# tchamp1912/Spittle

Measured on AMD Instinct MI355X. Metric: RTFx (audio-sec/wall-sec) Whisper-large-v3 30s chunks @1/2/4/8 MI355X, higher is better.
Workload: dtype bf16; 1 GPU; whisper-large-v3 30s chunks, batch 8/GPU, greedy en, 4-token prompt + 128 decode steps, host PCM in, text out; model=synthetic:large-v3, global_batch=8, seq_len=1500, decode_steps=128, parallelism=replicas x1 (utterance shards)

## Files before the change

include/spittle_hip.h:

```cpp
#ifndef SPITTLE_HIP_H
#define SPITTLE_HIP_H

#include <stddef.h>
#include <stdint.h>

#ifdef __cplusplus
extern "C" {
#endif

#define SPT_ABI_VERSION 14

typedef enum {
    SPT_OK = 0,
    SPT_ERR_INVALID_ARG = 1,
    SPT_ERR_LOAD = 2,
    SPT_ERR_DEVICE = 3,
    SPT_ERR_OOM = 4,
    SPT_ERR_UNSUPPORTED = 5,
    SPT_ERR_INTERNAL = 6
} spt_status;

typedef enum {
    SPT_DTYPE_F32 = 0, SPT_DTYPE_BF16 = 1,
    SPT_DTYPE_F16 = 2 ,
// ... 101 lines not shown
    int32_t decoder_passes;
    int32_t beam_steps;
    int32_t encoder_windows;
    double device_ms;
    double encoder_ms;
    double decode_ms;
    int32_t pd_passes;
    int32_t pd_fallbacks;
} spt_call_stats;

spt_status spt_get_call_stats(const spt_ctx* ctx, spt_call_stats* s);
spt_status spt_get_xq_stats(const spt_ctx* ctx, int32_t* fused_launches, int32_t* fallbacks);

spt_status spt_weights_export(spt_ctx* ctx, void* dev_dst, size_t bytes);
spt_status spt_weights_import(spt_ctx* ctx, const void* dev_src, size_t bytes);
spt_status spt_weights_arena(spt_ctx* ctx, void** dev_ptr, size_t* bytes);
spt_status spt_weights_commit(spt_ctx* ctx);

spt_status spt_ctx_create_replicas(const char* model_spec, const spt_model_params* params, const int32_t* devices,
                                   int32_t n_devices, spt_ctx** out, double* bcast_ms, char* err, size_t errlen);
spt_status spt_transcribe_batch_replicas(spt_ctx* const* ctxs, int32_t n_ctx, const float* const* pcm,
                                         const size_t* n_samples, size_t batch, const spt_infer_params* params,
                                         spt_result** out);

typedef enum {
    SPT_PROBE_DEC_CROSS_ATTN = 0,
    SPT_PROBE_DEC_SELF_ATTN = 1,
    SPT_PROBE_DEC_LOGITS = 2,
    SPT_PROBE_DEC_FC1 = 3,
    SPT_PROBE_ENC_FC1_GEMM = 4,
    SPT_PROBE_ENC_ATTN = 5
} spt_probe_kind;
spt_status spt_probe_kernel(spt_ctx* ctx, int32_t kind, int32_t iters, double* avg_us, double* work,
                            int32_t* work_is_flops);

spt_status spt_debug_mel(spt_ctx* ctx, const float* pcm16k, size_t n_samples, float* out);
spt_status spt_debug_mel_at(spt_ctx* ctx, const float* pcm16k, size_t n_samples, int32_t seek, float* out);
spt_status spt_debug_encode(spt_ctx* ctx, const float* mel, float* out);
spt_status spt_debug_weight_checksum(spt_ctx* ctx, int32_t tensor_id, double* out2);
spt_status spt_debug_ggml_tokenize(const char* model_path, const char* text, int32_t* tokens, int32_t n_max,
                                   int32_t* n_out);
spt_status spt_debug_ggml_dequant(int32_t ggml_type, const void* src, int64_t n, float* dst);
typedef struct {
    float temperature;
    int32_t suppress_blank;
    int32_t no_ts;
    int32_t max_initial;
    int32_t n_max;
    int32_t max_tokens;
    uint64_t seed;
} spt_sample_params;
spt_status spt_debug_sample_tokens(int32_t device, int32_t dtype, const float* logits, int32_t n_steps, int32_t B,
                                   int32_t n_vocab, int32_t ldl, int32_t eot, int32_t beg, int32_t blank,
                                   const uint32_t* suppress, const spt_sample_params* prm, const int32_t* seek,
                                   const int32_t* seek_end, int32_t* state, int32_t* done, const int32_t* forced,
                                   int32_t forced_len, int32_t out_cap, int32_t* dec_state, int32_t Tq, int32_t d,
                                   int32_t ctx, const float* emb, const float* pos, int32_t* out_tok, float* out_plog,
                                   float* out_tid, int32_t* next_tok, float* x, uint32_t* arrive, char* err,
                                   size_t errlen);
spt_status spt_debug_sample_beam(int32_t device, const float* logits, int32_t B, int32_t n_vocab, int32_t ldl,
                                 int32_t eot, int32_t beg, int32_t blank, const uint32_t* suppress,
                                 const spt_sample_params* prm, const int32_t* row, int32_t step, int32_t k,
                                 int32_t chunked, int32_t* cand_id, float* cand_lp, int32_t* tid, char* err,
                                 size_t errlen);
spt_status spt_debug_sample_kv_gather(int32_t device, int32_t dtype, const float* src, float* dst,
                                      const int32_t* rows, int32_t L, int32_t B, int32_t H, int32_t ctx,
                                      int32_t pos0, char* err, size_t errlen);
spt_status spt_debug_attn_enc(int32_t device, int32_t dtype, const float* qkv, int32_t B, int32_t T, int32_t H,
                              float* out, char* err, size_t errlen);
spt_status spt_debug_attn_self(int32_t device, int32_t dtype, const float* q, const float* cache, int32_t B,
                               int32_t H, int32_t ctx, int32_t Tq, int32_t pos0, float* out, char* err,
                               size_t errlen);
enum {
    SPT_ATTN_CROSS_8WAVE = 0,
    SPT_ATTN_CROSS_VW = 1,
    SPT_ATTN_CROSS_VW_PQ = 2,
    SPT_ATTN_CROSS_VW_MERGE = 3,
    SPT_ATTN_CROSS_VW_PQ_MERGE = 4
};
spt_status spt_debug_attn_cross(int32_t device, int32_t dtype, int32_t mode, const float* q, const float* k,
                                const float* v, float pad_value, int32_t B, int32_t B_layout, int32_t b0, int32_t H,
                                int32_t T_enc, int32_t Tq, int32_t splits, const int32_t* kvrow, int32_t share,
                                float* out, float* part, char* err, size_t errlen);

#define SPT_HAS_QUANT_RESIDENT 1
spt_status spt_get_weight_residency(const spt_ctx* ctx, int64_t* resident_weights, int64_t* resident_bytes,
                                    int32_t* ggml_type);
enum { SPT_GGML_Q4_1 = 3, SPT_GGML_Q5_0 = 6, SPT_GGML_Q5_1 = 7 };
enum { SPT_GV_BIAS = 0, SPT_GV_BIAS_GELU = 1, SPT_GV_PARTIAL = 2, SPT_GV_QKV_CACHE = 3, SPT_GV_LOGITS = 4,
       SPT_GV_BIAS_RESID = 5 };
enum { SPT_QGEMV_A_DIRECT = 0, SPT_QGEMV_A_LN = 1 };
spt_status spt_debug_qgemv(int32_t device, int32_t dtype, int32_t ggml_type, const void* blocks, size_t blocks_bytes,
                           int32_t N, int32_t K, const float* act, int32_t R, const float* ln_w, const float* ln_b,
                           const float* bias, const float* resid, int32_t mode, int32_t a_src, int32_t ksplit,
                           float* out_plain, float* out_packed, float* top_plain, float* top_packed, float* unpacked,
                           char* err, size_t errlen);

typedef struct spt_pk_ctx spt_pk_ctx;

typedef struct {
    int32_t dtype;
    int32_t device;
    int32_t max_batch;
    float max_seconds;
    uint64_t seed;
    uint32_t flags;
    int32_t reserved0;
} spt_pk_model_params;

#define SPT_PK_WEIGHTS_EMPTY 1u

typedef enum { SPT_PK_TS_TOKEN = 0, SPT_PK_TS_WORD = 1, SPT_PK_TS_SEGMENT = 2 } spt_pk_granularity;

typedef struct {
    int32_t max_symbols;
    int32_t timestamp_granularity;
} spt_pk_infer_params;

typedef struct {
    double start, end;
    char* text;
    int32_t i0, n_tokens;
} spt_pk_segment;

typedef struct {
    char* text;
    int32_t* tokens;
    int32_t* frames;
    float* logit;
    float* runner_up;
    int32_t n_tokens;
    int32_t n_segments;
    spt_pk_segment* segments;
    int32_t n_chunks;
    int32_t reserved0;
} spt_pk_result;

typedef struct {
    int32_t n_mels, d, n_layers, n_heads, ff, sub_ch, conv_k, pred, n_vocab, n_dur;
    int32_t dtype, max_batch, max_samples, reserved0;
    int64_t weight_bytes, workspace_bytes;
} spt_pk_model_info;

typedef struct {
    double mel_ms, encoder_ms, decode_ms, total_ms, h2d_ms;
    int32_t n_steps;
    int32_t batch;
    int32_t enc_frames;
    int32_t reserved0;
} spt_pk_timings;

void spt_parakeet_default_model_params(spt_pk_model_params* p);
void spt_parakeet_default_infer_params(spt_pk_infer_params* p);
spt_status spt_parakeet_create(const char* model_spec, const spt_pk_model_params* params, spt_pk_ctx** out,
                               char* err, size_t errlen);

typedef struct spt_pk_onnx spt_pk_onnx;
spt_status spt_parakeet_onnx_open(const char* dir, spt_pk_onnx** out, spt_pk_model_info* info, char* err, size_t errlen);
int64_t spt_parakeet_onnx_tensor(const spt_pk_onnx* h, int32_t tensor_id, const float** data);
int64_t spt_parakeet_onnx_qtensor(const spt_pk_onnx* h, int32_t tensor_id, const int16_t** q, const float** scales,
                                  const int32_t** zero_points, int32_t* n_scales);
const char* spt_parakeet_onnx_piece(const spt_pk_onnx* h, int32_t token_id);
void spt_parakeet_onnx_close(spt_pk_onnx* h);
void spt_parakeet_destroy(spt_pk_ctx* ctx);
const char* spt_parakeet_last_error(const spt_pk_ctx* ctx);
spt_status spt_parakeet_info(const spt_pk_ctx* ctx, spt_pk_model_info* info);
// ... 219 lines not shown
```

rust/spittle-hip-sys/src/lib.rs:

```rust
#![allow(non_camel_case_types)]

use std::os::raw::{c_char, c_int, c_void};

pub const SPT_ABI_VERSION: c_int = 14;
pub const SPT_PK_STAGE_COUNT: c_int = 9;

pub type spt_status = c_int;
pub const SPT_OK: spt_status = 0;
pub const SPT_ERR_INVALID_ARG: spt_status = 1;
pub const SPT_ERR_LOAD: spt_status = 2;
pub const SPT_ERR_DEVICE: spt_status = 3;
pub const SPT_ERR_OOM: spt_status = 4;
pub const SPT_ERR_UNSUPPORTED: spt_status = 5;
pub const SPT_ERR_INTERNAL: spt_status = 6;

pub type spt_dtype = c_int;
pub const SPT_DTYPE_F32: spt_dtype = 0;
pub const SPT_DTYPE_BF16: spt_dtype = 1;
pub const SPT_DTYPE_F16: spt_dtype = 2;
pub const SPT_DTYPE_I8: spt_dtype = 3;
pub const SPT_ATTN_CROSS_8WAVE: i32 = 0;
pub const SPT_ATTN_CROSS_VW: i32 = 1;
pub const SPT_ATTN_CROSS_VW_PQ: i32 = 2;
pub const SPT_ATTN_CROSS_VW_MERGE: i32 = 3;
// ... 288 lines not shown
    ) -> spt_status;
    pub fn spt_debug_sample_beam(
        device: i32,
        logits: *const f32,
        b: i32,
        n_vocab: i32,
        ldl: i32,
        eot: i32,
        beg: i32,
        blank: i32,
        suppress: *const u32,
        prm: *const spt_sample_params,
        row: *const i32,
        step: i32,
        k: i32,
        chunked: i32,
        cand_id: *mut i32,
        cand_lp: *mut f32,
        tid: *mut i32,
        err: *mut c_char,
        errlen: usize,
    ) -> spt_status;
    pub fn spt_debug_sample_kv_gather(
        device: i32,
        dtype: i32,
        src: *const f32,
        dst: *mut f32,
        rows: *const i32,
        l: i32,
        b: i32,
        h: i32,
        ctx: i32,
        pos0: i32,
        err: *mut c_char,
        errlen: usize,
    ) -> spt_status;
    pub fn spt_debug_attn_enc(
        device: i32,
        dtype: i32,
        qkv: *const f32,
        b: i32,
        t: i32,
        h: i32,
        out: *mut f32,
        err: *mut c_char,
        errlen: usize,
    ) -> spt_status;
    pub fn spt_debug_attn_self(
        device: i32,
        dtype: i32,
        q: *const f32,
        cache: *const f32,
        b: i32,
        h: i32,
        ctx: i32,
        tq: i32,
        pos0: i32,
        out: *mut f32,
        err: *mut c_char,
        errlen: usize,
    ) -> spt_status;
    pub fn spt_debug_attn_cross(
        device: i32,
        dtype: i32,
        mode: i32,
        q: *const f32,
        k: *const f32,
        v: *const f32,
        pad_value: f32,
        b: i32,
        b_layout: i32,
        b0: i32,
        h: i32,
        t_enc: i32,
        tq: i32,
        splits: i32,
        kvrow: *const i32,
        share: i32,
        out: *mut f32,
        part: *mut f32,
        err: *mut c_char,
        errlen: usize,
    ) -> spt_status;
    pub fn spt_get_weight_residency(
        ctx: *const spt_ctx,
        resident_weights: *mut i64,
        resident_bytes: *mut i64,
        ggml_type: *mut i32,
    ) -> spt_status;
    pub fn spt_debug_qgemv(
        device: i32,
        dtype: i32,
        ggml_type: i32,
        blocks: *const c_void,
        blocks_bytes: usize,
        n: i32,
        k: i32,
        act: *const f32,
        r: i32,
        ln_w: *const f32,
        ln_b: *const f32,
        bias: *const f32,
        resid: *const f32,
        mode: i32,
        a_src: i32,
        ksplit: i32,
        out_plain: *mut f32,
        out_packed: *mut f32,
        top_plain: *mut f32,
        top_packed: *mut f32,
        unpacked: *mut f32,
        err: *mut c_char,
        errlen: usize,
    ) -> spt_status;

    pub fn spt_parakeet_default_model_params(p: *mut spt_pk_model_params);
    pub fn spt_parakeet_default_infer_params(p: *mut spt_pk_infer_params);
    pub fn spt_parakeet_create(
        model_spec: *const c_char,
        params: *const spt_pk_model_params,
        out: *mut *mut spt_pk_ctx,
        err: *mut c_char,
        errlen: usize,
    ) -> spt_status;
    pub fn spt_parakeet_destroy(ctx: *mut spt_pk_ctx);
    pub fn spt_parakeet_last_error(ctx: *const spt_pk_ctx) -> *const c_char;
    pub fn spt_parakeet_info(ctx: *const spt_pk_ctx, info: *mut spt_pk_model_info) -> spt_status;
    pub fn spt_parakeet_tensor_numel(ctx: *const spt_pk_ctx, tensor_id: i32, n: *mut i64) -> spt_status;
    pub fn spt_parakeet_set_tensor(ctx: *mut spt_pk_ctx, tensor_id: i32, data: *const f32, n: i64) -> spt_status;
    pub fn spt_parakeet_set_vocab(ctx: *mut spt_pk_ctx, pieces: *const *const c_char, n: i32) -> spt_status;
    pub fn spt_parakeet_transcribe(
        ctx: *mut spt_pk_ctx,
        pcm16k: *const f32,
        n_samples: usize,
        params: *const spt_pk_infer_params,
        out: *mut *mut spt_pk_result,
    ) -> spt_status;
    pub fn spt_parakeet_transcribe_batch(
        ctx: *mut spt_pk_ctx,
        pcm: *const *const f32,
        n_samples: *const usize,
        batch: usize,
        params: *const spt_pk_infer_params,
        out: *mut *mut spt_pk_result,
    ) -> spt_status;
    pub fn spt_parakeet_transcribe_batch_device(
        ctx: *mut spt_pk_ctx,
        pcm_dev: *const f32,
        stride: usize,
        n_samples: *const usize,
        batch: usize,
        params: *const spt_pk_infer_params,
        out: *mut *mut spt_pk_result,
    ) -> spt_status;
    pub fn spt_parakeet_result_free(r: *mut spt_pk_result);
    pub fn spt_parakeet_get_timings(ctx: *const spt_pk_ctx, t: *mut spt_pk_timings) -> spt_status;
    pub fn spt_parakeet_profile_encoder(ctx: *mut spt_pk_ctx, iters: i32, ms: *mut f64, n: i32) -> spt_status;
    pub fn spt_parakeet_debug_mel(ctx: *mut spt_pk_ctx, pcm16k: *const f32, n_samples: usize, out: *mut f32) -> spt_status;
    pub fn spt_parakeet_debug_encode(ctx: *mut spt_pk_ctx, mel: *const f32, t: i32, out: *mut f32) -> spt_status;
    pub fn spt_parakeet_debug_last_encoder(ctx: *mut spt_pk_ctx, b: i32, out: *mut f32, t3: *mut i32) -> spt_status;
    pub fn spt_parakeet_debug_decode(
        ctx: *mut spt_pk_ctx,
        enc: *const f32,
        t3: i32,
        max_symbols: i32,
        out: *mut *mut spt_pk_result,
// ... 463 lines not shown
```

spittle_amd/_lib.py:

```python
from __future__ import annotations

import ctypes as C
import os

HERE = os.path.dirname(os.path.abspath(__file__))
LIB_PATH = os.path.join(HERE, "libspittle_hip.so")

SPT_OK, SPT_ERR_INVALID_ARG, SPT_ERR_LOAD, SPT_ERR_DEVICE, SPT_ERR_OOM, SPT_ERR_UNSUPPORTED, SPT_ERR_INTERNAL = range(7)
STATUS_NAMES = {0: "OK", 1: "INVALID_ARG", 2: "LOAD", 3: "DEVICE", 4: "OOM", 5: "UNSUPPORTED", 6: "INTERNAL"}
SPT_DTYPE_F32, SPT_DTYPE_BF16, SPT_DTYPE_F16, SPT_DTYPE_I8 = 0, 1, 2, 3
SPT_SUPPRESS_BLANK, SPT_NO_TIMESTAMPS, SPT_IGNORE_EOT, SPT_SUPPRESS_NST = 1, 2, 4, 8

EXPORTS = [
    "spt_version", "spt_default_model_params", "spt_default_infer_params", "spt_ctx_create",
    "spt_ctx_destroy", "spt_last_error", "spt_ctx_info", "spt_transcribe", "spt_transcribe_batch",
    "spt_transcribe_batch_device", "spt_result_free", "spt_get_timings", "spt_get_call_stats", "spt_get_xq_stats", "spt_debug_mel",
    "spt_debug_mel_at", "spt_debug_encode", "spt_debug_weight_checksum", "spt_probe_kernel", "spt_language_code",
    "spt_tokenize", "spt_token_to_str", "spt_debug_ggml_tokenize", "spt_debug_ggml_dequant",
    "spt_weights_export", "spt_weights_import", "spt_weights_arena", "spt_weights_commit",
    "spt_ctx_create_replicas", "spt_transcribe_batch_replicas",
    "spt_parakeet_default_model_params", "spt_parakeet_default_infer_params", "spt_parakeet_create",
    "spt_parakeet_destroy", "spt_parakeet_last_error", "spt_parakeet_info", "spt_parakeet_tensor_numel",
    "spt_parakeet_set_tensor", "spt_parakeet_set_vocab", "spt_parakeet_transcribe", "spt_parakeet_transcribe_batch",
    "spt_parakeet_transcribe_batch_device", "spt_parakeet_result_free", "spt_parakeet_get_timings",
    "spt_parakeet_debug_mel", "spt_parakeet_debug_encode", "spt_parakeet_debug_decode", "spt_parakeet_debug_last_encoder",
    "spt_parakeet_debug_weight_checksum", "spt_parakeet_onnx_open", "spt_parakeet_onnx_tensor",
    "spt_parakeet_onnx_piece", "spt_parakeet_onnx_close",
    "spt_resampler_create", "spt_resampler_info", "spt_resample_output_len", "spt_resample",
    "spt_resampler_last_error", "spt_resampler_destroy",
    "spt_vad_default_params", "spt_vad_create", "spt_vad_push", "spt_vad_result_free", "spt_vad_reset",
    "spt_vad_last_error", "spt_vad_destroy",
    "spt_parakeet_profile_encoder",
    "spt_parakeet_onnx_qtensor", "spt_parakeet_debug_qgemm", "spt_parakeet_debug_tap", "spt_parakeet_debug_tap_read",
    "spt_moonshine_default_model_params", "spt_moonshine_default_infer_params", "spt_moonshine_create",
    "spt_moonshine_destroy", "spt_moonshine_last_error", "spt_moonshine_info", "spt_moonshine_tensor_numel",
    "spt_moonshine_set_tensor", "spt_moonshine_missing_tensors", "spt_moonshine_set_vocab", "spt_moonshine_transcribe",
    "spt_moonshine_transcribe_batch", "spt_moonshine_result_free", "spt_moonshine_get_timings",
    "spt_moonshine_debug_stem", "spt_moonshine_debug_encode", "spt_moonshine_debug_logits",
    "spt_sensevoice_default_model_params", "spt_sensevoice_default_infer_params", "spt_sensevoice_create",
    "spt_sensevoice_destroy", "spt_sensevoice_last_error", "spt_sensevoice_info", "spt_sensevoice_tensor_numel",
    "spt_sensevoice_set_tensor", "spt_sensevoice_missing_tensors", "spt_sensevoice_set_cmvn",
    "spt_sensevoice_set_vocab", "spt_sensevoice_n_rows", "spt_sensevoice_transcribe",
    "spt_sensevoice_transcribe_batch", "spt_sensevoice_result_free", "spt_sensevoice_get_timings",
    "spt_sensevoice_debug_features", "spt_sensevoice_debug_encode", "spt_sensevoice_debug_frames",
    "spt_debug_sample_tokens", "spt_debug_sample_beam", "spt_debug_sample_kv_gather",
    "spt_debug_attn_enc", "spt_debug_attn_self", "spt_debug_attn_cross",
    "spt_debug_qgemv", "spt_get_weight_residency",
]
SPT_MODEL_QUANT_RESIDENT = 2
SPT_GGML_Q4_1, SPT_GGML_Q5_0, SPT_GGML_Q5_1 = 3, 6, 7
SPT_GV_BIAS, SPT_GV_BIAS_GELU, SPT_GV_PARTIAL, SPT_GV_QKV_CACHE, SPT_GV_LOGITS, SPT_GV_BIAS_RESID = range(6)
SPT_QGEMV_A_DIRECT, SPT_QGEMV_A_LN = 0, 1
SPT_ATTN_CROSS_8WAVE, SPT_ATTN_CROSS_VW, SPT_ATTN_CROSS_VW_PQ, SPT_ATTN_CROSS_VW_MERGE, SPT_ATTN_CROSS_VW_PQ_MERGE = range(5)
SPT_SV_LANG_AUTO, SPT_SV_LANG_ZH, SPT_SV_LANG_EN, SPT_SV_LANG_YUE, SPT_SV_LANG_JA, SPT_SV_LANG_KO = range(6)
SPT_PK_WEIGHTS_EMPTY = 1
SPT_PK_TS_TOKEN, SPT_PK_TS_WORD, SPT_PK_TS_SEGMENT = 0, 1, 2
SPT_MODEL_WEIGHTS_EXTERNAL = 1
PK_STAGES = ("subsampling", "pos", "layernorm", "ffn", "qkv_out", "attn", "conv_pw", "conv_dw", "joint_enc")
PROBES = {"dec_cross_attn": 0, "dec_self_attn": 1, "dec_logits": 2, "dec_fc1": 3, "enc_fc1_gemm": 4,
          "enc_attn": 5}


class ModelParams(C.Structure):
    _fields_ = [("dtype", C.c_int32), ("device", C.c_int32), ("max_batch", C.c_int32),
                ("flags", C.c_uint32), ("seed", C.c_uint64)]


class InferParams(C.Structure):
    _fields_ = [("language", C.c_char_p), ("translate", C.c_int32), ("initial_prompt", C.c_char_p),
                ("flags", C.c_uint32), ("max_new_tokens", C.c_int32), ("temperature", C.c_float),
                ("beam_size", C.c_int32), ("forced_tokens", C.POINTER(C.c_int32)), ("n_forced", C.c_int32),
                ("prompt_tokens", C.POINTER(C.c_int32)), ("n_prompt_tokens", C.c_int32),
                ("temperature_inc", C.c_float), ("best_of", C.c_int32), ("entropy_thold", C.c_float),
                ("logprob_thold", C.c_float), ("max_initial_ts", C.c_float), ("reserved0", C.c_int32),
                ("seed", C.c_uint64)]


class Segment(C.Structure):
    _fields_ = [("t0", C.c_int64), ("t1", C.c_int64), ("text", C.c_char_p), ("i0", C.c_int32),
                ("n_tokens", C.c_int32)]


class Result(C.Structure):
    _fields_ = [("text", C.c_char_p), ("tokens", C.POINTER(C.c_int32)), ("top1", C.POINTER(C.c_float)),
                ("top2", C.POINTER(C.c_float)), ("n_tokens", C.c_int32), ("n_windows", C.c_int32),
                ("language", C.c_int32), ("n_segments", C.c_int32), ("segments", C.POINTER(Segment)),
                ("n_fallbacks", C.c_int32), ("reserved0", C.c_int32)]


class ModelInfo(C.Structure):
    _fields_ = [(n, C.c_int32) for n in ("n_mels", "d", "n_head", "n_enc", "n_dec", "n_vocab", "n_audio_ctx",
                                          "n_text_ctx", "dtype", "max_batch")] + \
               [("weight_bytes", C.c_int64), ("workspace_bytes", C.c_int64)]


class Timings(C.Structure):
    _fields_ = [(n, C.c_double) for n in ("mel_ms", "encoder_ms", "cross_kv_ms", "decode_ms", "total_ms",
                                           "h2d_ms")] + [("n_decode_passes", C.c_int32), ("batch", C.c_int32)]


class CallStats(C.Structure):
    _fields_ = [(n, C.c_int32) for n in ("engine_calls", "decoder_passes", "beam_steps", "encoder_windows")] + \
               [(n, C.c_double) for n in ("device_ms", "encoder_ms", "decode_ms")] + \
               [(n, C.c_int32) for n in ("pd_passes", "pd_fallbacks")]


class PkModelParams(C.Structure):
    _fields_ = [("dtype", C.c_int32), ("device", C.c_int32), ("max_batch", C.c_int32), ("max_seconds", C.c_float),
                ("seed", C.c_uint64), ("flags", C.c_uint32), ("reserved0", C.c_int32)]


class PkInferParams(C.Structure):
    _fields_ = [("max_symbols", C.c_int32), ("timestamp_granularity", C.c_int32)]


class PkSegment(C.Structure):
    _fields_ = [("start", C.c_double), ("end", C.c_double), ("text", C.c_char_p), ("i0", C.c_int32),
                ("n_tokens", C.c_int32)]


class PkResult(C.Structure):
    _fields_ = [("text", C.c_char_p), ("tokens", C.POINTER(C.c_int32)), ("frames", C.POINTER(C.c_int32)),
                ("logit", C.POINTER(C.c_float)), ("runner_up", C.POINTER(C.c_float)), ("n_tokens", C.c_int32),
                ("n_segments", C.c_int32), ("segments", C.POINTER(PkSegment)), ("n_chunks", C.c_int32),
                ("reserved0", C.c_int32)]


class PkModelInfo(C.Structure):
    _fields_ = [(n, C.c_int32) for n in ("n_mels", "d", "n_layers", "n_heads", "ff", "sub_ch", "conv_k", "pred",
# ... 193 lines not shown
    L.spt_vad_result_free.restype = None
    L.spt_vad_reset.argtypes = [vp, C.c_int32]
    L.spt_vad_reset.restype = C.c_int
    L.spt_vad_last_error.argtypes = [vp]
    L.spt_vad_last_error.restype = C.c_char_p
    L.spt_vad_destroy.argtypes = [vp]
    L.spt_vad_destroy.restype = None
    MR = C.POINTER(C.POINTER(MsResult))
    L.spt_moonshine_default_model_params.argtypes = [C.POINTER(MsModelParams)]
    L.spt_moonshine_default_model_params.restype = None
    L.spt_moonshine_default_infer_params.argtypes = [C.POINTER(MsInferParams)]
    L.spt_moonshine_default_infer_params.restype = None
    L.spt_moonshine_create.argtypes = [C.c_char_p, C.POINTER(MsModelParams), C.POINTER(vp), C.c_char_p, C.c_size_t]
    L.spt_moonshine_destroy.argtypes = [vp]
    L.spt_moonshine_destroy.restype = None
    L.spt_moonshine_last_error.argtypes = [vp]
    L.spt_moonshine_last_error.restype = C.c_char_p
    L.spt_moonshine_info.argtypes = [vp, C.POINTER(MsModelInfo)]
    L.spt_moonshine_tensor_numel.argtypes = [vp, C.c_char_p, C.POINTER(C.c_int64)]
    L.spt_moonshine_set_tensor.argtypes = [vp, C.c_char_p, fp, C.c_int64]
    L.spt_moonshine_missing_tensors.argtypes = [vp]
    L.spt_moonshine_missing_tensors.restype = C.c_int32
    L.spt_moonshine_set_vocab.argtypes = [vp, C.POINTER(C.c_char_p), C.c_int32]
    L.spt_moonshine_transcribe.argtypes = [vp, fp, C.c_size_t, C.POINTER(MsInferParams), MR]
    L.spt_moonshine_transcribe_batch.argtypes = [vp, C.POINTER(fp), C.POINTER(C.c_size_t), C.c_size_t,
                                                 C.POINTER(MsInferParams), MR]
    L.spt_moonshine_result_free.argtypes = [C.POINTER(MsResult)]
    L.spt_moonshine_result_free.restype = None
    L.spt_moonshine_get_timings.argtypes = [vp, C.POINTER(MsTimings)]
    L.spt_moonshine_debug_stem.argtypes = [vp, fp, C.c_size_t, fp]
    L.spt_moonshine_debug_encode.argtypes = [vp, fp, C.c_size_t, fp]
    L.spt_moonshine_debug_logits.argtypes = [vp, fp, C.c_size_t, i32p, C.c_int32, fp]
    for fn in ("spt_moonshine_create", "spt_moonshine_info", "spt_moonshine_tensor_numel", "spt_moonshine_set_tensor",
               "spt_moonshine_set_vocab", "spt_moonshine_transcribe", "spt_moonshine_transcribe_batch",
               "spt_moonshine_get_timings", "spt_moonshine_debug_stem", "spt_moonshine_debug_encode",
               "spt_moonshine_debug_logits"):
        getattr(L, fn).restype = C.c_int
    SR = C.POINTER(C.POINTER(SvResult))
    svip = C.POINTER(SvInferParams)
    L.spt_sensevoice_default_model_params.argtypes = [C.POINTER(SvModelParams)]
    L.spt_sensevoice_default_model_params.restype = None
    L.spt_sensevoice_default_infer_params.argtypes = [svip]
    L.spt_sensevoice_default_infer_params.restype = None
    L.spt_sensevoice_create.argtypes = [C.c_char_p, C.POINTER(SvModelParams), C.POINTER(vp), C.c_char_p, C.c_size_t]
    L.spt_sensevoice_destroy.argtypes = [vp]
    L.spt_sensevoice_destroy.restype = None
    L.spt_sensevoice_last_error.argtypes = [vp]
    L.spt_sensevoice_last_error.restype = C.c_char_p
    L.spt_sensevoice_info.argtypes = [vp, C.POINTER(SvModelInfo)]
    L.spt_sensevoice_tensor_numel.argtypes = [vp, C.c_char_p, C.POINTER(C.c_int64)]
    L.spt_sensevoice_set_tensor.argtypes = [vp, C.c_char_p, fp, C.c_int64]
    L.spt_sensevoice_missing_tensors.argtypes = [vp]
    L.spt_sensevoice_missing_tensors.restype = C.c_int32
    L.spt_sensevoice_set_cmvn.argtypes = [vp, fp, fp, C.c_int32]
    L.spt_sensevoice_set_vocab.argtypes = [vp, C.POINTER(C.c_char_p), C.c_int32]
    L.spt_sensevoice_n_rows.argtypes = [vp, C.c_size_t]
    L.spt_sensevoice_n_rows.restype = C.c_int32
    L.spt_sensevoice_transcribe.argtypes = [vp, fp, C.c_size_t, svip, SR]
    L.spt_sensevoice_transcribe_batch.argtypes = [vp, C.POINTER(fp), C.POINTER(C.c_size_t), C.c_size_t, svip, SR]
    L.spt_sensevoice_result_free.argtypes = [C.POINTER(SvResult)]
    L.spt_sensevoice_result_free.restype = None
    L.spt_sensevoice_get_timings.argtypes = [vp, C.POINTER(SvTimings)]
    L.spt_sensevoice_debug_features.argtypes = [vp, fp, C.c_size_t, fp]
    L.spt_sensevoice_debug_encode.argtypes = [vp, fp, C.c_size_t, svip, fp]
    L.spt_sensevoice_debug_frames.argtypes = [vp, fp, C.c_size_t, svip, i32p, fp, fp]
    for fn in ("spt_sensevoice_create", "spt_sensevoice_info", "spt_sensevoice_tensor_numel", "spt_sensevoice_set_tensor",
               "spt_sensevoice_set_cmvn", "spt_sensevoice_set_vocab", "spt_sensevoice_transcribe",
               "spt_sensevoice_transcribe_batch", "spt_sensevoice_get_timings", "spt_sensevoice_debug_features",
               "spt_sensevoice_debug_encode", "spt_sensevoice_debug_frames"):
        getattr(L, fn).restype = C.c_int
    u32p, spp, i32 = C.POINTER(C.c_uint32), C.POINTER(SampleParams), C.c_int32
    L.spt_debug_sample_tokens.argtypes = [i32, i32, fp, i32, i32, i32, i32, i32, i32, i32, u32p, spp, i32p, i32p, i32p,
                                          i32p, i32p, i32, i32, i32p, i32, i32, i32, fp, fp, i32p, fp, fp, i32p, fp,
                                          u32p, C.c_char_p, C.c_size_t]
    L.spt_debug_sample_beam.argtypes = [i32, fp, i32, i32, i32, i32, i32, i32, u32p, spp, i32p, i32, i32, i32, i32p, fp,
                                        i32p, C.c_char_p, C.c_size_t]
    L.spt_debug_sample_kv_gather.argtypes = [i32, i32, fp, fp, i32p, i32, i32, i32, i32, i32, C.c_char_p, C.c_size_t]
    for fn in ("spt_debug_sample_tokens", "spt_debug_sample_beam", "spt_debug_sample_kv_gather"):
        getattr(L, fn).restype = C.c_int
    L.spt_debug_attn_enc.argtypes = [i32, i32, fp, i32, i32, i32, fp, C.c_char_p, C.c_size_t]
    L.spt_debug_attn_self.argtypes = [i32, i32, fp, fp, i32, i32, i32, i32, i32, fp, C.c_char_p, C.c_size_t]
    L.spt_debug_attn_cross.argtypes = [i32, i32, i32, fp, fp, fp, C.c_float, i32, i32, i32, i32, i32, i32, i32, i32p,
                                       i32, fp, fp, C.c_char_p, C.c_size_t]
    for fn in ("spt_debug_attn_enc", "spt_debug_attn_self", "spt_debug_attn_cross"):
        getattr(L, fn).restype = C.c_int
    L.spt_debug_qgemv.argtypes = [i32, i32, i32, C.c_void_p, C.c_size_t, i32, i32, fp, i32, fp, fp, fp, fp, i32, i32,
                                  i32, fp, fp, fp, fp, fp, C.c_char_p, C.c_size_t]
    L.spt_debug_qgemv.restype = C.c_int
    L.spt_get_weight_residency.argtypes = [vp, C.POINTER(C.c_int64), C.POINTER(C.c_int64), C.POINTER(C.c_int32)]
    L.spt_get_weight_residency.restype = C.c_int
    for fn in EXPORTS:
        if fn.startswith("spt_parakeet_") and fn not in ("spt_parakeet_default_model_params",
                                                          "spt_parakeet_default_infer_params", "spt_parakeet_destroy",
                                                          "spt_parakeet_last_error", "spt_parakeet_result_free",
                                                          "spt_parakeet_onnx_tensor", "spt_parakeet_onnx_piece",
                                                          "spt_parakeet_onnx_close", "spt_parakeet_onnx_qtensor"):
            getattr(L, fn).restype = C.c_int
    for fn in ("spt_weights_arena", "spt_weights_commit", "spt_ctx_create_replicas", "spt_transcribe_batch_replicas",
               "spt_weights_export", "spt_weights_import", "spt_ctx_info", "spt_transcribe", "spt_transcribe_batch", "spt_transcribe_batch_device",
               "spt_get_timings", "spt_get_call_stats", "spt_get_xq_stats", "spt_debug_mel", "spt_debug_mel_at", "spt_debug_encode", "spt_debug_weight_checksum",
               "spt_probe_kernel", "spt_tokenize", "spt_debug_ggml_tokenize", "spt_debug_ggml_dequant"):
        getattr(L, fn).restype = C.c_int
    _lib = L
    return L
```

spittle_amd/attn_debug.py:

```python
from __future__ import annotations

import ctypes as C

import numpy as np

from . import _lib as L
from .engine import TranscriptionError

DTYPES = {"f32": L.SPT_DTYPE_F32, "bf16": L.SPT_DTYPE_BF16, "f16": L.SPT_DTYPE_F16}
MODES = {"8wave": L.SPT_ATTN_CROSS_8WAVE, "vw": L.SPT_ATTN_CROSS_VW, "vw_pq": L.SPT_ATTN_CROSS_VW_PQ,
         "vw_merge": L.SPT_ATTN_CROSS_VW_MERGE, "vw_pq_merge": L.SPT_ATTN_CROSS_VW_PQ_MERGE}


def _ptr(x, t=C.c_float):
    return None if x is None else x.ctypes.data_as(C.POINTER(t))


def _check(st, err):
    if st != L.SPT_OK:
        raise TranscriptionError(st, err.value.decode())


def enc(qkv, B, T, H, dtype="f32", device: int = 0) -> np.ndarray:
    lib = L.load()
    x = None if qkv is None else np.ascontiguousarray(qkv, np.float32)
    if x is not None and x.size != B * T * 3 * H * 64:
        raise ValueError("enc: qkv is [B*T][3*H*64]")
    out = np.zeros((max(B * T, 1), max(H, 1) * 64), np.float32)
    err = C.create_string_buffer(512)
    _check(lib.spt_debug_attn_enc(device, DTYPES[dtype], _ptr(x), B, T, H, _ptr(out), err, 512), err)
    return out


def self_attn(q, cache, pos0, Tq, dtype="f32", device: int = 0) -> np.ndarray:
    lib = L.load()
    c = np.ascontiguousarray(cache, np.float32)
    two, B, H, ctx, hd = c.shape
    if two != 2 or hd != 64:
        raise ValueError("self_attn: cache is [2][B][H][ctx][64]")
    x = np.ascontiguousarray(q, np.float32)
    if x.size != B * max(Tq, 0) * H * 64 and 1 <= Tq <= 4:
        raise ValueError("self_attn: q is [B*Tq][H*64]")
    out = np.zeros((B * max(Tq, 1), H * 64), np.float32)
    err = C.create_string_buffer(512)
    _check(lib.spt_debug_attn_self(device, DTYPES[dtype], _ptr(x), _ptr(c), B, H, ctx, Tq, pos0, _ptr(out), err, 512),
           err)
    return out


def cross(q, k, v, *, Tq=1, mode="8wave", splits=1, b0=0, B=None, kvrow=None, share=1, pad_value=0.0, dtype="f32",
          device: int = 0) -> np.ndarray:
    lib = L.load()
    kk = np.ascontiguousarray(k, np.float32)
    vv = np.ascontiguousarray(v, np.float32)
    B_layout, H, T_enc, hd = kk.shape
    if hd != 64 or vv.shape != kk.shape:
        raise ValueError("cross: k and v are [B_layout][H][T_enc][64]")
    x = np.ascontiguousarray(q, np.float32)
    if B is None:
        B = x.size // (max(Tq, 1) * H * 64)
    if 1 <= Tq <= 4 and x.size != B * Tq * H * 64:
        raise ValueError("cross: q is [B*Tq][H*64]")
    km = None if kvrow is None else np.ascontiguousarray(kvrow, np.int32)
    if km is not None and km.shape != (B,):
        raise ValueError("cross: one window per row")
    m = MODES[mode] if isinstance(mode, str) else int(mode)
    R = max(B * max(Tq, 1), 1)
    vw = m >= L.SPT_ATTN_CROSS_VW
    want_part = (vw and m not in (L.SPT_ATTN_CROSS_VW_MERGE, L.SPT_ATTN_CROSS_VW_PQ_MERGE)) or (not vw and splits > 1)
    out = np.zeros((R, H * 64), np.float32)
    part = np.zeros((R, H, 8 if vw else max(min(splits, 4), 1), 66), np.float32)
    err = C.create_string_buffer(512)
    st = lib.spt_debug_attn_cross(device, DTYPES[dtype], m, _ptr(x), _ptr(kk), _ptr(vv), float(pad_value), B, B_layout,
                                  b0, H, T_enc, Tq, splits, _ptr(km, C.c_int32), share, _ptr(out), _ptr(part), err, 512)
    _check(st, err)
    return part if want_part else out
```

spittle_amd/csrc/capi_attn.cpp:

```cpp
#include <hip/hip_runtime.h>
#include <string.h>

#include <stdexcept>
#include <string>
#include <vector>

#include "../../include/spittle_hip.h"
#include "capi_debug.h"
#include "capi_internal.h"
#include "common.h"
#include "kernels.h"

namespace {

using namespace spt::dbg;

const void* up_as(Scope& sc, int dtype, const float* v, size_t n, std::vector<uint16_t>& h16) {
    if (dtype == spt::DT_F32) return sc.up(v, n);
    h16 = to_half_storage(dtype, v, n);
    return sc.up(h16.data(), n);
}

void down_f32(Scope& sc, int dtype, const void* dev, float* h, size_t n) {
    if (dtype == spt::DT_F32) {
// ... 89 lines not shown
    }
}

spt_status spt_debug_attn_cross(int32_t device, int32_t dtype, int32_t mode, const float* q, const float* k,
                                const float* v, float pad_value, int32_t B, int32_t B_layout, int32_t b0, int32_t H,
                                int32_t T_enc, int32_t Tq, int32_t splits, const int32_t* kvrow, int32_t share,
                                float* out, float* part, char* err, size_t errlen) {
    if (!q || !k || !v) {
        set_err(err, errlen, "null argument");
        return SPT_ERR_INVALID_ARG;
    }
    const bool vw = mode >= SPT_ATTN_CROSS_VW;
    const bool per_query = mode == SPT_ATTN_CROSS_VW_PQ || mode == SPT_ATTN_CROSS_VW_PQ_MERGE;
    const bool merge = mode == SPT_ATTN_CROSS_VW_MERGE || mode == SPT_ATTN_CROSS_VW_PQ_MERGE;
    try {
        check_dtype(dtype);
        if (mode < SPT_ATTN_CROSS_8WAVE || mode > SPT_ATTN_CROSS_VW_PQ_MERGE) throw std::runtime_error("debug_attn_cross: mode 0..4");
        if (B < 1 || B > 1024 || H < 1 || B_layout < 1) throw std::runtime_error("debug_attn_cross: need 1..1024 rows, H, B_layout >= 1");
        if (T_enc < 1) throw std::runtime_error("debug_attn_cross: T_enc below 1");
        if (Tq < 1 || Tq > 4) throw std::runtime_error("dec_cross_attn: 1..4 queries per sequence");
        if (splits < 1 || splits > 4) throw std::runtime_error("dec_cross_attn: 1..4 key chunks");
        if (splits > 1 && vw) throw std::runtime_error("debug_attn_cross: key chunks are the 8-wave kernel's");
        if (share < 1 || share > 8 || B % share) throw std::runtime_error("dec_cross_attn: rows per window 1..8, dividing B");
        if (share > 1 && !kvrow) throw std::runtime_error("dec_cross_attn: shared windows need the window map");
        if (per_query && Tq != 1) throw std::runtime_error("debug_attn_cross: per_query is the one-token step's");
        const int nq = share * Tq;
        const int NQ = nq == 1 ? 1 : Tq > 1 ? 4 : (spt::dtype_size(dtype) == 2 ? 5 : 4);
        if (splits > 1 && nq > NQ) throw std::runtime_error("dec_cross_attn: key chunks need one query chunk per window");
        if ((int64_t)((T_enc + 31) / 32) * B_layout * H * 4096 >= (int64_t)INT32_MAX)
            throw std::runtime_error("dec_cross_attn: a layer's cross K/V exceeds 2^31 elements");
        if (spt::kv_layer_elems(B_layout, H, T_enc) > kMaxElems || (int64_t)B * Tq * H * 66 * 8 > kMaxElems)
            throw std::runtime_error("debug_attn_cross: buffers above 2^26 elements");
        if (b0 < 0 || (int64_t)b0 + B / share > B_layout) throw std::runtime_error("debug_attn_cross: b0 + B / share beyond B_layout");
        if (kvrow)
            for (int i = 0; i < B; ++i)
                if (kvrow[i] < 0 || (int64_t)b0 + kvrow[i] >= B_layout)
                    throw std::runtime_error("debug_attn_cross: window map entry outside the layout");
        const bool wants_part = (vw && !merge) || (!vw && splits > 1);
        if (wants_part ? !part : !out) throw std::runtime_error("debug_attn_cross: null output for this mode");
    } catch (const std::exception& e) {
        set_err(err, errlen, e.what());
        return SPT_ERR_INVALID_ARG;
    }
    if (spt_status s = device_ok(device, err, errlen)) return s;
    try {
        const size_t n_kv = (size_t)spt::kv_layer_elems(B_layout, H, T_enc);
        std::vector<float> lay(n_kv, pad_value);
        const int T32 = (T_enc + 31) / 32 * 32;
        for (int kvi = 0; kvi < 2; ++kvi) {
            const float* src = kvi ? v : k;
            for (int b = 0; b < B_layout; ++b)
                for (int h = 0; h < H; ++h)
                    for (int t = 0; t < T32; ++t) {
                        float* dst = lay.data() + spt::kv_offset(0, kvi, b, h, t, 0, B_layout, H, T_enc);
                        if (t < T_enc) memcpy(dst, src + (((size_t)b * H + h) * T_enc + t) * 64, 64 * sizeof(float));
                    }
        }
        const size_t R = (size_t)B * Tq, nq_el = R * H * 64, esz = (size_t)spt::dtype_size(dtype);
        const int S = vw ? 8 : splits;
        const size_t n_part = R * H * S * 66;
        std::vector<uint16_t> q16, kv16;
        Scope sc(device);
        const void* d_q = up_as(sc, dtype, q, nq_el, q16);
        const char* d_kv = (const char*)up_as(sc, dtype, lay.data(), n_kv, kv16) + (size_t)b0 * H * 4096 * esz;
        const int* d_map = kvrow ? sc.up(kvrow, (size_t)B) : nullptr;
        float* d_part = (vw || splits > 1) ? sc.out<float>(n_part) : nullptr;
        void* d_out = (!vw && splits == 1) || merge ? sc.out<char>(nq_el * esz) : nullptr;
        if (vw) {
            spt::dec_cross_attn_vw(dtype, d_q, d_kv, B, B_layout, H, T_enc, Tq, d_part, sc.st, d_map, share, per_query);
            if (merge) spt::dec_attn_part_merge(dtype, d_part, (int)R, H, d_out, sc.st);
        } else {
            spt::dec_cross_attn(dtype, d_q, d_kv, B, B_layout, H, T_enc, Tq, d_out, sc.st, splits, d_part, d_map, share);
        }
        if (d_out) down_f32(sc, dtype, d_out, out, nq_el);
        else sc.down(part, (const float*)d_part, n_part);
        sc.sync();
        return SPT_OK;
    } catch (const std::exception& e) {
        set_err(err, errlen, e.what());
        return spt_classify(e);
    }
}

}
```

spittle_amd/csrc/dec_attn.h:

```cpp
#pragma once
#include "common.h"

namespace spt {
namespace {

constexpr int AW = 8;
constexpr float kLog2Scale = 0.125f * 1.4426950408889634f;

template <typename T> struct KVChunk;
template <> struct KVChunk<bf16> {
    bf16x8 v;
    __device__ __forceinline__ void load(const bf16* p) { v = *(const bf16x8*)p; }
    __device__ __forceinline__ float at(int e) const { return bf2f((bf16)v[e]); }
};
template <> struct KVChunk<f16> {
    f16x8 v;
    __device__ __forceinline__ void load(const f16* p) { v = *(const f16x8*)p; }
    __device__ __forceinline__ float at(int e) const { return (float)v[e]; }
};
template <> struct KVChunk<float> {
    f32x4 a, b;
    __device__ __forceinline__ void load(const float* p) { a = *(const f32x4*)p; b = *(const f32x4*)(p + 4); }
    __device__ __forceinline__ float at(int e) const { return e < 4 ? a[e] : b[e - 4]; }
};
// ... 68 lines not shown
#pragma unroll
                for (int e = 0; e < 8; ++e) o[t][e] = __builtin_fmaf(p, vc[i].at(e), o[t][e]);
            }
            l[t] = __builtin_fmaf(l[t], alpha, ls);
            m[t] = mn;
        }
    }
    template <int MAXB>
    __device__ __forceinline__ void run(int blk, int nblk, const float (&qv)[NQ][8], const int (&lim)[NQ], int Tq) {
        if (blk >= nblk) return;
        const int cnt = (nblk - 1 - blk) / NW + 1;
        const int mine = blk + (cnt - 1) * NW;
        if (MAXB <= 8 && cnt <= MAXB) {
#pragma unroll
            for (int d = 0; d < PF - 1 && d < MAXB; ++d) load_blk(kc_[d], vc_[d], min(blk + d * NW, mine));
#pragma unroll
            for (int i = 0; i < (MAXB <= 8 ? MAXB : 1); ++i) {
                if (i >= cnt) break;
                if (i + PF - 1 < (MAXB <= 8 ? MAXB : 1))
                    load_blk(kc_[(i + PF - 1) % PF], vc_[(i + PF - 1) % PF], min(blk + (i + PF - 1) * NW, mine));
                process(kc_[i % PF], vc_[i % PF], (blk + i * NW) * KB, qv, lim, Tq);
            }
            return;
        }
        load_blk(kc_[0], vc_[0], blk);
        while (blk < nblk) {
            load_blk(kc_[1], vc_[1], min(blk + NW, mine));
            process(kc_[0], vc_[0], blk * KB, qv, lim, Tq);
            blk += NW;
            if (blk >= nblk) break;
            load_blk(kc_[0], vc_[0], min(blk + NW, mine));
            process(kc_[1], vc_[1], blk * KB, qv, lim, Tq);
            blk += NW;
        }
    }
    template <int MAXB>
    __device__ __forceinline__ void run_pre(int blk, int nblk, const float (&qv)[NQ][8], const int (&lim)[NQ], int Tq) {
        if (blk >= nblk) return;
        const int cnt = (nblk - 1 - blk) / NW + 1;
        const int mine = blk + (cnt - 1) * NW;
        if (MAXB <= 8 && cnt <= MAXB) {
#pragma unroll
            for (int d = 1; d < PF - 1 && d < MAXB; ++d) load_blk(kc_[d], vc_[d], min(blk + d * NW, mine));
#pragma unroll
            for (int i = 0; i < (MAXB <= 8 ? MAXB : 1); ++i) {
                if (i >= cnt) break;
                if (i + PF - 1 < (MAXB <= 8 ? MAXB : 1))
                    load_blk(kc_[(i + PF - 1) % PF], vc_[(i + PF - 1) % PF], min(blk + (i + PF - 1) * NW, mine));
                process(kc_[i % PF], vc_[i % PF], (blk + i * NW) * KB, qv, lim, Tq);
            }
            return;
        }
        while (blk < nblk) {
            load_blk(kc_[1], vc_[1], min(blk + NW, mine));
            process(kc_[0], vc_[0], blk * KB, qv, lim, Tq);
            blk += NW;
            if (blk >= nblk) break;
            load_blk(kc_[0], vc_[0], min(blk + NW, mine));
            process(kc_[1], vc_[1], blk * KB, qv, lim, Tq);
            blk += NW;
        }
    }
    template <int MAXB>
    __device__ __forceinline__ void ring_fill(int blk, int nblk) {
        static_assert(MAXB <= 8, "AttnWave: ring_fill / ring_run are the unrolled schedule");
        const int cnt = blk < nblk ? (nblk - 1 - blk) / NW + 1 : 1;
        const int mine = blk + (cnt - 1) * NW;
#pragma unroll
        for (int d = 0; d < PF - 1 && d < MAXB; ++d) load_blk(kc_[d], vc_[d], min(blk + d * NW, mine));
    }
    template <int MAXB>
    __device__ __forceinline__ void ring_run(int blk, int nblk, const float (&qv)[NQ][8], const int (&lim)[NQ], int Tq) {
        if (blk >= nblk) return;
        const int cnt = (nblk - 1 - blk) / NW + 1;
        const int mine = blk + (cnt - 1) * NW;
#pragma unroll
        for (int i = 0; i < MAXB; ++i) {
            if (i >= cnt) break;
            if (i + PF - 1 < MAXB)
                load_blk(kc_[(i + PF - 1) % PF], vc_[(i + PF - 1) % PF], min(blk + (i + PF - 1) * NW, mine));
            process(kc_[i % PF], vc_[i % PF], (blk + i * NW) * KB, qv, lim, Tq);
        }
    }
    __device__ __forceinline__ void to_lds(float (*s_m)[NQ], float (*s_l)[NQ], float (*s_o)[NQ][64], int wid,
                                           int lane) {
        const int g = lane & 7;
#pragma unroll
        for (int t = 0; t < NQ; ++t) {
            float lt = l[t];
            lt += __shfl_xor(lt, 8, 64);
            lt += __shfl_xor(lt, 16, 64);
            lt += __shfl_xor(lt, 32, 64);
#pragma unroll
            for (int e = 0; e < 8; ++e) {
                float v = o[t][e];
                v += __shfl_xor(v, 8, 64);
                v += __shfl_xor(v, 16, 64);
                v += __shfl_xor(v, 32, 64);
                o[t][e] = v;
            }
            if (lane < 8) {
#pragma unroll
                for (int e = 0; e < 8; ++e) s_o[wid][t][8 * g + e] = o[t][e];
            }
            if (lane == 0) {
                s_m[wid][t] = m[t];
                s_l[wid][t] = lt;
            }
        }
    }
};

template <int NQ, int NW = AW>
__device__ __forceinline__ void attn_merge(const float (*s_m)[NQ], const float (*s_l)[NQ], const float (*s_o)[NQ][64],
                                           int t, int e, float& M, float& L, float& O) {
#pragma clang fp contract(off)
    M = -INFINITY;
#pragma unroll
    for (int w = 0; w < NW; ++w) M = fmaxf(M, s_m[w][t]);
    L = 0.f;
    O = 0.f;
#pragma unroll
    for (int w = 0; w < NW; ++w) {
        if (s_m[w][t] == -INFINITY) continue;
        const float f = exp2f(s_m[w][t] - M);
        L = __builtin_fmaf(s_l[w][t], f, L);
        O = __builtin_fmaf(s_o[w][t][e], f, O);
    }
}

}
}
```

spittle_amd/csrc/engine.cpp:

```cpp
#include "engine.h"
#include "ggml_file.h"
#include "ggml_qpack.h"

#include <cstdio>

#include <math.h>
#include <string.h>

#include <algorithm>
#include <functional>
#include <cstdlib>
#include <sstream>
#include <stdexcept>

#include "common.h"

namespace spt {

bool parse_synthetic_spec(const std::string& spec, ModelDims* dm, uint64_t* seed, std::string* err) {
    const std::string pfx = "synthetic:";
    if (spec.compare(0, pfx.size(), pfx) != 0) return false;
    std::vector<std::string> parts;
    std::stringstream ss(spec.substr(pfx.size()));
    std::string tok;
// ... 874 lines not shown
}

void Engine::run_cross_kv(int B) {
    const int d = dm_.d, T = dm_.n_audio_ctx;
    GemmArgs g{};
    g.A = enc_out_; g.lda = d; g.W = ckv_w_; g.ldw = d; g.M = B * T; g.N = dm_.n_dec * 2 * d; g.K = d;
    g.bias = ckv_b_; g.C = ckv_; g.kv_B = B; g.kv_T = T; g.kv_H = dm_.n_head;
    gemm_nt(dt_, EPI_KVSPLIT, g, 1, st_);
}

void Engine::enqueue_decoder_pass(DecGroup& g, int E, int Tq, const DecodeRequest& rq, int out_cap) {
    float* x = enqueue_layers(g, E, Tq);
    enqueue_head(g, Tq, rq, out_cap, x, suppress_, (rq.flags & 1u) != 0);
}

float* Engine::enqueue_layers(DecGroup& g, int E, int Tq) {
    const int d = dm_.d, H = dm_.n_head, ctx = dm_.n_text_ctx, T = dm_.n_audio_ctx, B = g.B, R = B * Tq;
    const int64_t self_layer = (int64_t)2 * B * H * ctx * 64, cross_layer = kv_layer_elems(E, H, T);
    const bool mapped = g.share > 0;
    const int runs = B / std::max(1, g.share);
    const int vw_env = getenv("SPT_XATTN_VW") ? atoi(getenv("SPT_XATTN_VW")) : 1;
    const bool vw = vw_env == 2 || (vw_env != 0 && runs * H < 96);
    const bool per_query = vw && Tq == 1 && vw_env != 3;
    const bool vw_merge = vw && R > 1;
    const int xs = vw ? (vw_merge ? 1 : 8) : mapped ? 1 : xsplit_;
    const int ks = esz_ == 2 ? 128 : 64;
    hipStream_t st = g.st;
    const bool fuse = xq_on_ && probe_kind_ < 0 && Tq == 1 && !vw && !mapped && xs == 1 && dm_.n_dec <= 64 &&
                      dec_xq_fused_ok(dt_, B, d, H, T, n_cu_);
    xq_enq_ = fuse ? dm_.n_dec : 0;
    if (fuse) {
        hipStreamCaptureStatus cap = hipStreamCaptureStatusNone;
        HIP_CHECK(hipStreamIsCapturing(st, &cap));
        if (cap == hipStreamCaptureStatusNone) cs_.xq_fused += xq_enq_;
    }
    float* xc = g.dx;
    float* xo = g.dx2;
    int np = 0;
    pend_fold_ = !getenv("SPT_DEC_XFOLD") || atoi(getenv("SPT_DEC_XFOLD")) != 0;
    auto ln_input = [&](GemvArgs& a) {
        ln_source(a, xc, g.pend, np, (int64_t)R * d);
        a.x_out = np > 0 ? xo : nullptr;
    };
    auto consumed = [&] {
        if (np > 0) std::swap(xc, xo);
        np = 0;
    };
    auto pmark = [&](int kind, int l, int which) {
        if (probe_kind_ == kind) HIP_CHECK(hipEventRecord(probe_ev_[2 * l + which], st));
    };
    auto partial = [&](GemvArgs& a, int split) {
        a.C = g.pend; a.ldc = d; a.c_split = (int64_t)R * d;
        a.ksplit = split;
        a.p_resid = pend_fold_ ? xc : nullptr;
        if (a.K / ks < split) throw std::runtime_error("decoder projection too narrow for its K split");
        np = split;
    };
    for (int l = 0; l < dm_.n_dec; ++l) {
        const DecL& e = dec_[l];
        void* skv_l = (char*)g.skv + self_layer * l * esz_;
        const void* ckv_l = (const char*)ckv_ + (cross_layer * l + (mapped ? 0 : (int64_t)g.b0 * H * 4096)) * esz_;
        {
            GemvArgs a{};
            ln_input(a); a.lda = d; a.ln_w = e.ln1_w; a.ln_b = e.ln1_b; a.R = R;
            a.W = e.qkv_w; a.wq = e.qkv_q; a.N = 3 * d; a.K = d; a.bias = e.qkv_b; a.C = g.dq; a.ldc = d;
            a.cache = skv_l; a.cache_B = B; a.cache_H = H; a.cache_ctx = ctx; a.Tq = Tq; a.st = g.ds;
            gemv(dt_, GV_QKV_CACHE, A_LN, a, st);
            consumed();
            pmark(1, l, 0);
            dec_self_attn(dt_, g.dq, skv_l, B, H, ctx, Tq, g.ds, g.dao, st);
            pmark(1, l, 1);
        }
        GemvArgs a{};
        a.A = g.dao; a.lda = d; a.R = R; a.W = e.so_w; a.wq = e.so_q; a.N = d; a.K = d; a.bias = e.so_b;
        a.C = xc; a.ldc = d;
        gemv(dt_, GV_BIAS_RESID, A_DIRECT, a, st);
        a = GemvArgs{};
        ln_input(a); a.lda = d; a.ln_w = e.ln2_w; a.ln_b = e.ln2_b; a.R = R;
        a.W = e.cq_w; a.wq = e.cq_q; a.N = d; a.K = d; a.bias = e.cq_b; a.C = g.dq; a.ldc = d;
        if (fuse) {
            if (np != 0) throw std::runtime_error("fused cross-Q launch: pending slabs before LN2");
            XqFuseArgs x{};
            x.kv = ckv_l; x.B_layout = E; x.H = H; x.T_enc = T; x.out = g.dao; x.gran = g.xq_gran; x.ds = g.ds;
            x.err = xq_err_; x.layer = l;
            dec_xq_fused(dt_, a, x, B, st);
        } else {
            gemv(dt_, GV_BIAS, A_LN, a, st);
        }
        consumed();
        pmark(0, l, 0);
        if (fuse) {
        } else if (vw) {
            dec_cross_attn_vw(dt_, g.dq, ckv_l, B, E, H, T, Tq, g.xpart, st, mapped ? g.kvrow : nullptr,
                              mapped ? g.share : 1, per_query);
            if (vw_merge) dec_attn_part_merge(dt_, g.xpart, R, H, g.dao, st);
        }
        else
            dec_cross_attn(dt_, g.dq, ckv_l, B, E, H, T, Tq, g.dao, st, xs, g.xpart, mapped ? g.kvrow : nullptr,
                           mapped ? g.share : 1);
        pmark(0, l, 1);
        a = GemvArgs{};
        a.A = g.dao; a.lda = d; a.R = R; a.W = e.co_w; a.wq = e.co_q; a.N = d; a.K = d; a.bias = e.co_b; a.C = xc; a.ldc = d;
        if (xs > 1) { a.apart = g.xpart; a.a_splits = xs; a.a_heads = H; }
        gemv(dt_, GV_BIAS_RESID, xs > 1 ? A_ATTN : A_DIRECT, a, st);
        a = GemvArgs{};
        ln_input(a); a.lda = d; a.ln_w = e.ln3_w; a.ln_b = e.ln3_b; a.R = R;
        a.W = e.fc1_w; a.wq = e.fc1_q; a.N = 4 * d; a.K = d; a.bias = e.fc1_b; a.C = g.dff; a.ldc = 4 * d;
        pmark(3, l, 0);
        gemv(dt_, GV_BIAS_GELU, A_LN, a, st);
        pmark(3, l, 1);
        consumed();
        a = GemvArgs{};
        a.A = g.dff; a.lda = 4 * d; a.R = R; a.W = e.fc2_w; a.wq = e.fc2_q; a.N = d; a.K = 4 * d; a.bias = e.fc2_b;
        partial(a, fc2_split_);
        gemv(dt_, GV_PARTIAL, A_DIRECT, a, st);
    }
    return xc;
}

void Engine::ln_source(GemvArgs& a, float* xc, float* pend, int np, int64_t slab) const {
    const int f = np > 0 && pend_fold_ ? 1 : 0;
    a.A = f ? pend : xc;
    for (int p = 0; p < kMaxPend; ++p) a.pend[p] = p < np - f ? pend + (int64_t)(p + f) * slab : zero_;
    a.n_pend = np - f;
}

void Engine::enqueue_head(DecGroup& g, int Tq, const DecodeRequest& rq, int out_cap, float* xc,
                          const uint32_t* sup, bool blank) {
    const int d = dm_.d, ctx = dm_.n_text_ctx, B = g.B, R = B * Tq;
    hipStream_t st = g.st;
    const Specials sp = specials_for(dm_.n_vocab);
    const int n_tiles = (dm_.n_vocab + 15) / 16;
    GemvArgs a{};
    ln_source(a, xc, g.pend, fc2_split_, (int64_t)R * d);
    a.lda = Tq * d; a.a_row0 = (Tq - 1) * d; a.ln_w = lnf_w_; a.ln_b = lnf_b_; a.R = B;
    a.W = tok_emb_; a.wq = tok_q_; a.N = dm_.n_vocab; a.K = d; a.C = g.logits; a.ldc = dm_.n_vocab; a.st = g.ds;
    a.suppress = sup;
    a.blank0 = blank ? sp.eot : -1;
    a.blank1 = blank ? 220 : -1;
    a.part = g.part; a.n_tiles = n_tiles;
    gemv(dt_, GV_LOGITS, A_LN, a, st);
    if (rq.beam_k > 0) {
        BeamArgs bm{};
        bm.logits = g.logits; bm.ldl = dm_.n_vocab;
        bm.n_vocab = dm_.n_vocab; bm.eot = sp.eot; bm.beg = sp.beg; bm.blank = rq.blank_tok;
        bm.suppress = sup; bm.prm = g.prm; bm.row = g.beam_row; bm.step = g.beam_step; bm.k = rq.beam_k;
        bm.cand_id = g.cand_id; bm.cand_lp = g.cand_lp; bm.tid = g.beam_tid;
        static const bool one_wg = getenv("SPT_BEAM_ONE_WG") != nullptr;
        bm.stat = one_wg ? nullptr : g.beam_stat;
        dec_beam_topk(bm, B, st);
        dec_advance(g.ds, Tq, st);
        return;
    }
    if (rq.full) {
        TsArgs t{};
        t.logits = g.logits; t.ldl = dm_.n_vocab;
        t.n_vocab = dm_.n_vocab; t.eot = sp.eot; t.beg = sp.beg; t.blank = rq.blank_tok;
        t.suppress = sup; t.prm = g.prm; t.seek = g.seek; t.seek_end = g.seek_end; t.state = g.ts_state;
        t.forced = rq.n_forced > 0 ? g.forced : nullptr; t.forced_len = rq.n_forced;
        t.next_tok = g.tok_in; t.out_tok = g.out_tok; t.out_plog = g.out_t1; t.out_tid = g.out_t2; t.out_cap = out_cap;
        t.done = g.done;
        t.emb = tok_emb_; t.emb_q = tok_q_; t.pos = dec_pos_; t.d = d; t.ctx = ctx; t.Tq = Tq; t.x = g.dx;
        t.ds = g.ds; t.arrive = g.arrive; t.stat = g.ts_stat;
        dec_ts_stats(t, B, st);
        dec_finalize_ts(dt_, t, B, st);
        return;
    }
// ... 148 lines not shown
            ~XqRestore() { on = v; }
        } xq_restore{xq_on_, xq_on};
        for (DecGroup* g : act) {
            reset_outputs(*g);
            upload_tokens(*g, [&](int, int) { return sp.sot; }, 1);
            dec_embed(dt_, g->tok_in, g->B, 1, dm_.d, tok_emb_, tok_q_, dec_pos_, g->ds, g->dx, g->st);
            float* x = enqueue_layers(*g, E, 1);
            enqueue_head(*g, 1, dq, out_cap, x, suppress_lang_, false);
        }
        std::vector<int> first((size_t)B * out_cap);
        for (DecGroup* g : act) {
            HIP_CHECK(hipMemcpyAsync(first.data() + (size_t)g->b0 * out_cap, g->out_tok, (size_t)g->B * out_cap * 4,
                                     hipMemcpyDeviceToHost, g->st));
            HIP_CHECK(hipStreamSynchronize(g->st));
        }
        for (int b = 0; b < B; ++b) {
            const int v = rq.lang_tok[b];
            lang[b] = v >= 0 ? v : first[(size_t)(-v - 1) * out_cap];
            if (lang[b] <= sp.sot || lang[b] > sp.sot + sp.n_langs) throw std::runtime_error("language detection failed");
        }
    } else if (!rq.lang_tok.empty()) {
        for (int b = 0; b < B; ++b) lang[b] = rq.lang_tok[b];
    }
    if (lang_out)
        for (int b = 0; b < B; ++b) lang_out[b] = lang[b] >= 0 ? lang[b] : (Tq >= 3 ? rq.prompt[1] : -1);
    for (DecGroup* gp : act) {
        DecGroup& g = *gp;
        reset_outputs(g);
        const bool rows = !rq.row_prefix.empty();
        const int P = rows ? (int)rq.row_prefix[0].size() : (int)rq.prefix.size();
        for (int c0 = 0; c0 < P; c0 += cmax) {
            const int n = std::min(cmax, P - c0);
            upload_tokens(g, [&](int b, int t) { return rows ? rq.row_prefix[b][c0 + t] : rq.prefix[c0 + t]; }, n);
            dec_embed(dt_, g.tok_in, g.B * n, n, dm_.d, tok_emb_, tok_q_, dec_pos_, g.ds, g.dx, g.st);
            enqueue_layers(g, E, n);
            dec_advance(g.ds, n, g.st);
        }
        auto prompt_tok = [&](int b, int t) { return (t == 1 && lang[b] >= 0) ? lang[b] : rq.prompt[t]; };
        for (int c0 = 0; c0 < Tq - Tq_head; c0 += cmax) {
            const int n = std::min(cmax, Tq - Tq_head - c0);
            upload_tokens(g, [&](int b, int t) { return prompt_tok(b, c0 + t); }, n);
            dec_embed(dt_, g.tok_in, g.B * n, n, dm_.d, tok_emb_, tok_q_, dec_pos_, g.ds, g.dx, g.st);
            enqueue_layers(g, E, n);
            dec_advance(g.ds, n, g.st);
        }
        upload_tokens(g, [&](int b, int t) { return prompt_tok(b, Tq - Tq_head + t); }, Tq_head);
        dec_embed(dt_, g.tok_in, g.B * Tq_head, Tq_head, dm_.d, tok_emb_, tok_q_, dec_pos_, g.ds, g.dx, g.st);
        if (rq.beam_k > 0) {
            beam_host_.assign((size_t)g.B * 4 + 1, 0);
            for (int b = 0; b < g.B; ++b) beam_host_[b * 4 + 3] = 3000;
            HIP_CHECK(hipMemcpyAsync(g.beam_row, beam_host_.data(), (size_t)g.B * 16, hipMemcpyHostToDevice, g.st));
            HIP_CHECK(hipMemcpyAsync(g.beam_step, beam_host_.data() + (size_t)g.B * 4, 4, hipMemcpyHostToDevice, g.st));
        }
        enqueue_decoder_pass(g, E, Tq_head, rq, out_cap);
    }
    if (rq.beam_k > 0) {
        tm_.n_decode_passes = 1;
        for (DecGroup* g : act) {
            HIP_CHECK(hipEventRecord(g->ev, g->st));
            HIP_CHECK(hipStreamWaitEvent(st_, g->ev, 0));
        }
        return;
    }
    int passes = 1;
    static const bool no_graph = getenv("SPT_NO_GRAPH") != nullptr;
    static const bool sync_debug = getenv("SPT_DEBUG_SYNC") != nullptr;
    if (rq.n_steps > 1 && no_graph) {
        for (int s = 1; s < rq.n_steps; ++s, ++passes)
            for (DecGroup* g : act) {
                enqueue_decoder_pass(*g, E, 1, rq, out_cap);
                if (!sync_debug) continue;
                const hipError_t e = hipStreamSynchronize(g->st);
                DecState h{};
                if (e == hipSuccess) HIP_CHECK(hipMemcpy(&h, g->ds, sizeof(h), hipMemcpyDeviceToHost));
                if (e != hipSuccess || h.step != s + 1 || (s % 16) == 0)
                    fprintf(stderr, "[spt] pass %d: %s step=%d pos0=%d\n", s, hipGetErrorString(e), h.step, h.pos0);
                if (e != hipSuccess) throw HipError(std::string("pass failed: ") + hipGetErrorString(e));
            }
    } else if (rq.n_steps > 1) {
        std::vector<PassGraph> ex;
        for (DecGroup* g : act) {
            GraphKey key{g->B, E, g->b0, out_cap, rq.n_forced, rq.flags, rq.full};
            key.share = S;
            key.fuse = xq_on_;
            auto it = g->graphs.find(key);
            if (it == g->graphs.end()) {
                hipGraph_t graph;
                HIP_CHECK(hipStreamBeginCapture(g->st, hipStreamCaptureModeThreadLocal));
                enqueue_decoder_pass(*g, E, 1, rq, out_cap);
                HIP_CHECK(hipStreamEndCapture(g->st, &graph));
                hipGraphExec_t exec;
                HIP_CHECK(hipGraphInstantiate(&exec, graph, nullptr, nullptr, 0));
                HIP_CHECK(hipGraphDestroy(graph));
                it = g->graphs.emplace(key, PassGraph{exec, xq_enq_}).first;
            }
            ex.push_back(it->second);
        }
        const bool early_exit = !(rq.flags & 4u);
        std::vector<int> hdone(B);
        for (int s = 1; s < rq.n_steps; ++s) {
            for (size_t i = 0; i < act.size(); ++i) {
                HIP_CHECK(hipGraphLaunch(ex[i].exec, act[i]->st));
                cs_.xq_fused += ex[i].fused;
            }
            ++passes;
            if (early_exit && (s % 16) == 0) {
                bool all = true;
                for (DecGroup* g : act) {
                    HIP_CHECK(hipMemcpyAsync(hdone.data(), g->done, g->B * 4, hipMemcpyDeviceToHost, g->st));
                    HIP_CHECK(hipStreamSynchronize(g->st));
                    all = all && std::all_of(hdone.begin(), hdone.begin() + g->B, [](int v) { return v != 0; });
                }
                if (all) break;
            }
        }
    }
    tm_.n_decode_passes = passes;
    for (DecGroup* g : act) {
        const size_t off = (size_t)g->b0 * out_cap, n = (size_t)g->B * out_cap * 4;
        HIP_CHECK(hipMemcpyAsync(tokens + off, g->out_tok, n, hipMemcpyDeviceToHost, g->st));
        if (top1) HIP_CHECK(hipMemcpyAsync(top1 + off, g->out_t1, n, hipMemcpyDeviceToHost, g->st));
        if (top2) HIP_CHECK(hipMemcpyAsync(top2 + off, g->out_t2, n, hipMemcpyDeviceToHost, g->st));
        if (ts_state_out && rq.full)
            HIP_CHECK(hipMemcpyAsync(ts_state_out + (size_t)g->b0 * 4, g->ts_state, (size_t)g->B * 16,
                                     hipMemcpyDeviceToHost, g->st));
        HIP_CHECK(hipEventRecord(g->ev, g->st));
        HIP_CHECK(hipStreamWaitEvent(st_, g->ev, 0));
    }
}

void Engine::decode(int B, const DecodeRequest& rq, int* tokens, float* top1, float* top2, int* lang_out,
                    int* ts_state_out) {
    select();
    require_weights();
    const char* xq_env = getenv("SPT_XQ_FUSE");
    xq_on_ = rq.beam_k == 0 && !(xq_env && atoi(xq_env) == 0);
    struct XqOff {
        bool& on;
        ~XqOff() { on = false; }
    } xq_off{xq_on_};
    const int fused0 = cs_.xq_fused;
    HIP_CHECK(hipEventRecord(ev_[6], st_));
    run_decode(B, rq, tokens, top1, top2, lang_out, ts_state_out);
    HIP_CHECK(hipEventRecord(ev_[7], st_));
    HIP_CHECK(hipStreamSynchronize(st_));
    HIP_CHECK(hipGetLastError());
    if (cs_.xq_fused > fused0) {
        unsigned err = 0;
        HIP_CHECK(hipMemcpy(&err, xq_err_, 4, hipMemcpyDeviceToHost));
        const char* force = getenv("SPT_XQ_FUSE_FORCE_FALLBACK");
        if (err || (force && atoi(force) != 0)) {
            HIP_CHECK(hipMemset(xq_err_, 0, 4));
            xq_on_ = false;
            cs_.xq_fallbacks++;
            HIP_CHECK(hipEventRecord(ev_[6], st_));
            run_decode(B, rq, tokens, top1, top2, lang_out, ts_state_out);
            HIP_CHECK(hipEventRecord(ev_[7], st_));
            HIP_CHECK(hipStreamSynchronize(st_));
            HIP_CHECK(hipGetLastError());
        }
    }
    tm_.batch = B;
    cs_.engine_calls++;
    cs_.decoder_passes += tm_.n_decode_passes;
    finish_call_timing();
}

void Engine::finish_call_timing() {
    float ms;
    HIP_CHECK(hipEventElapsedTime(&ms, ev_[6], ev_[7]));
    tm_.decode_ms = ms;
    double total = ms;
    if (enc_pending_) {
        float m_norm, m_enc, m_kv;
        HIP_CHECK(hipEventElapsedTime(&m_norm, ev_[2], ev_[3]));
        HIP_CHECK(hipEventElapsedTime(&m_enc, ev_[3], ev_[4]));
        HIP_CHECK(hipEventElapsedTime(&m_kv, ev_[4], ev_[5]));
        tm_.encoder_ms = m_enc;
        tm_.cross_kv_ms = m_kv;
        tm_.mel_ms = m_norm;
        cs_.encoder_ms += m_enc;
        total += m_norm + m_enc + m_kv;
    } else {
        tm_.encoder_ms = tm_.cross_kv_ms = tm_.mel_ms = 0.0;
    }
    if (mel_pending_) {
        HIP_CHECK(hipEventElapsedTime(&ms, ev_[0], ev_[1]));
        tm_.mel_ms += ms;
        total += ms;
    }
    tm_.total_ms = total;
    cs_.device_ms += total;
    cs_.decode_ms += tm_.decode_ms;
    mel_pending_ = enc_pending_ = false;
}

void Engine::transcribe_device(const float* pcm_dev, int64_t stride, const int* n_samples, int B,
                               const DecodeRequest& rq, int* tokens, float* top1, float* top2, int* lang_out,
                               int* ts_state_out) {
    if (B < 1 || B > max_batch_) throw std::runtime_error("batch exceeds the context's max_batch");
    for (int b = 0; b < B; ++b)
        if (n_samples[b] < 0 || n_samples[b] > 480000 || (int64_t)n_samples[b] > stride)
            throw std::runtime_error("each window must hold 0..480000 samples within its stride");
    load_utterances_device(pcm_dev, stride, n_samples, B);
    std::vector<int> utt(B), seek(B, 0);
    for (int b = 0; b < B; ++b) utt[b] = b;
    encode_windows(utt.data(), seek.data(), B);
    decode(B, rq, tokens, top1, top2, lang_out, ts_state_out);
}

void Engine::transcribe_host(const float* const* pcm, const int* n_samples, int B, const DecodeRequest& rq,
                             int* tokens, float* top1, float* top2, int* lang_out, int* ts_state_out) {
    if (B < 1 || B > max_batch_) throw std::runtime_error("batch exceeds the context's max_batch");
    for (int b = 0; b < B; ++b)
        if (n_samples[b] < 0 || n_samples[b] > 480000) throw std::runtime_error("window longer than 30 s");
    load_utterances(pcm, n_samples, B);
    std::vector<int> utt(B), seek(B, 0);
    for (int b = 0; b < B; ++b) utt[b] = b;
    encode_windows(utt.data(), seek.data(), B);
// ... 329 lines not shown
```

spittle_amd/csrc/engine.h:

```cpp
#pragma once
#include <hip/hip_runtime.h>
#include <stdint.h>

#include <map>
#include <set>
#include <string>
#include <vector>

#include "kernels.h"
#include "vocab.h"

namespace spt {

class GgmlFile;

struct ModelDims {
    std::string name;
    int n_mels = 80, d = 384, n_head = 6, n_enc = 4, n_dec = 4, n_vocab = 51864;
    int n_audio_ctx = 1500, n_text_ctx = 448;
};


struct DecodeRequest {
    std::vector<int> prompt;
// ... 6 lines not shown
    bool full = false;
    TsParams ts{};
    std::vector<int> seek, seek_end;
    std::vector<std::vector<int>> row_prefix;
    std::vector<int> extra_suppress;
    int blank_tok = 220;
    int beam_k = 0;
    std::vector<int> kv_row;
};

struct BeamCands {
    std::vector<int> id;
    std::vector<float> lp;
    std::vector<int> tid;
};

struct Timings {
    double mel_ms = 0, encoder_ms = 0, cross_kv_ms = 0, decode_ms = 0, total_ms = 0, h2d_ms = 0;
    int n_decode_passes = 0, batch = 0;
};

struct CallStats {
    int engine_calls = 0, decoder_passes = 0, beam_steps = 0, encoder_windows = 0;
    int pd_passes = 0;
    int pd_fallbacks = 0;
    int xq_fused = 0;
    int xq_fallbacks = 0;
    double device_ms = 0, encoder_ms = 0, decode_ms = 0;
};

class Engine {
public:
    Engine(const ModelDims& dm, int dtype, int device, int max_batch, uint64_t seed, const GgmlFile* src = nullptr,
           bool external_weights = false, bool quant_resident = false);
    ~Engine();
    Engine(const Engine&) = delete;
    Engine& operator=(const Engine&) = delete;

    const ModelDims& dims() const { return dm_; }
    int dtype() const { return dt_; }
    int max_batch() const { return max_batch_; }
    int max_rows() const { return max_rows_; }
    int64_t weight_bytes() const { return wbytes_; }
    void weight_residency(int64_t* weights, int64_t* bytes, int* type) const {
        *weights = res_weights_; *bytes = res_bytes_; *type = res_type_;
    }
    bool weights_ready() const { return weights_ready_; }
    void export_weights(void* dev_dst, int64_t bytes);
    void import_weights(const void* dev_src, int64_t bytes);
    void* weight_arena() const { return warena_; }
    int device() const { return dev_; }
    void commit_weights();
    int64_t workspace_bytes() const { return abytes_; }
    const Timings& timings() const { return tm_; }
    const CallStats& call_stats() const { return cs_; }
    void reset_call_stats() { cs_ = CallStats(); }

    void load_utterances(const float* const* pcm_host, const int* n, int U);
    void load_utterances_device(const float* pcm_dev, int64_t stride, const int* n, int U);
    void encode_windows(const int* utt, const int* seek, int E);
    int encoded_windows() const { return enc_E_; }
    void decode(int B, const DecodeRequest& rq, int* tokens, float* top1, float* top2, int* lang_out = nullptr,
                int* ts_state_out = nullptr);

    void transcribe_device(const float* pcm_dev, int64_t stride, const int* n_samples, int B, const DecodeRequest& rq,
                           int* tokens, float* top1, float* top2, int* lang_out = nullptr, int* ts_state_out = nullptr);
    void transcribe_host(const float* const* pcm, const int* n_samples, int B, const DecodeRequest& rq, int* tokens,
                         float* top1, float* top2, int* lang_out = nullptr, int* ts_state_out = nullptr);

    void beam_begin(int B, const DecodeRequest& rq, BeamCands* out, int* lang_out);
    void beam_next(const int* src, const int* tokens, const int* rowstate, int step, BeamCands* out);

    void debug_mel(const float* pcm_host, int n, int seek, float* out_host);
    void debug_encode(const float* mel_host, float* out_host);
    bool debug_weight_checksum(int tid, double* out2);
    double probe(int kind, int iters, double* work, int* is_flops);

private:
    struct GraphKey {
        int B, B_total, b0, out_cap, n_forced;
        uint32_t flags;
        bool full;
        int share = 0;
        bool fuse = false;
        bool operator<(const GraphKey& o) const {
            if (full != o.full) return full < o.full;
            if (fuse != o.fuse) return fuse < o.fuse;
            if (B != o.B) return B < o.B;
            if (share != o.share) return share < o.share;
            if (B_total != o.B_total) return B_total < o.B_total;
            if (b0 != o.b0) return b0 < o.b0;
            if (out_cap != o.out_cap) return out_cap < o.out_cap;
            if (n_forced != o.n_forced) return n_forced < o.n_forced;
            return flags < o.flags;
        }
    };
    struct PassGraph {
        hipGraphExec_t exec;
        int fused;
    };
    struct DecGroup {
        hipStream_t st = nullptr;
        hipEvent_t ev = nullptr;
        int b0 = 0, B = 0;
        float* dx = nullptr;
        void *dq = nullptr, *dao = nullptr, *dff = nullptr;
        void* skv = nullptr;
        float* logits = nullptr;
        void* part = nullptr;
        unsigned* arrive = nullptr;
        int *tok_in = nullptr, *out_tok = nullptr, *done = nullptr, *forced = nullptr;
        float *out_t1 = nullptr, *out_t2 = nullptr;
        DecState* ds = nullptr;
        float* dx2 = nullptr;
        float* pend = nullptr;
        float* xpart = nullptr;
        int *seek = nullptr, *seek_end = nullptr, *ts_state = nullptr;
        float* ts_stat = nullptr;
        float* beam_stat = nullptr;
        TsParams* prm = nullptr;
        int *beam_row = nullptr, *beam_step = nullptr, *beam_src = nullptr;
        int *cand_id = nullptr, *beam_tid = nullptr;
        float* cand_lp = nullptr;
        int* kvrow = nullptr;
        int share = 0;
        unsigned long long* xq_gran = nullptr;
        std::map<GraphKey, PassGraph> graphs;
        std::vector<int> host_tok;
        size_t host_used = 0;
    };

    void select() const;
    void release();
    void alloc_weights();
    void generate_weights();
    void load_ggml(const GgmlFile& f);
    void alloc_workspace();
    void upload_tables(const std::vector<float>* filters);
    void run_mel_utts(const float* pcm, const std::vector<int64_t>& pcm_off, const int* n, int U);
    void upload_windows(const int* utt, const int* seek, int E);
    void finish_call_timing();
    void run_encoder(int B);
    void enc_layer(int l, int Bg, int64_t r0, hipStream_t s, int probe = 0, hipEvent_t e0 = nullptr,
                   hipEvent_t e1 = nullptr);
    int enc_groups_cur_ = 1;
    void enqueue_encoder(int B);
    void run_cross_kv(int B);
    void run_decode(int B, const DecodeRequest& rq, int* tokens, float* top1, float* top2, int* lang_out,
                    int* ts_state_out);
    void enqueue_decoder_pass(DecGroup& g, int E, int Tq, const DecodeRequest& rq, int out_cap);
    float* enqueue_layers(DecGroup& g, int E, int Tq);
    void enqueue_head(DecGroup& g, int Tq, const DecodeRequest& rq, int out_cap, float* xc, const uint32_t* sup,
                      bool blank);

    ModelDims dm_;
    int dt_, dev_, max_batch_;
    uint64_t seed_;
    int esz_;
    int cp_;
    static constexpr int fc2_split_ = 2;
    bool pend_fold_ = true;
    void ln_source(GemvArgs& a, float* xc, float* pend, int np, int64_t slab) const;
    bool xq_on_ = false;
    int xq_enq_ = 0;
    int n_cu_ = 0;
    unsigned* xq_err_ = nullptr;
    int xsplit_ = 1;
    int n_groups_ = 1;
    int max_rows_ = 64;
    hipStream_t st_ = nullptr;
    std::vector<hipEvent_t> ev_;
    static constexpr int kEncGroupsMax = 4;
    std::vector<hipStream_t> enc_st_;
    std::vector<hipEvent_t> enc_ev_;
    int enc_groups(int B) const;
    int probe_kind_ = -1;
    std::vector<hipEvent_t> probe_ev_;

    char* warena_ = nullptr;
    int64_t wbytes_ = 0;
    bool weights_ready_ = false;
    void require_weights() const;
    struct EncL { float *ln1_w, *ln1_b; void* qkv_w; float* qkv_b; void* o_w; float* o_b; float *ln2_w, *ln2_b;
                  void* fc1_w; float* fc1_b; void* fc2_w; float* fc2_b; };
    struct DecL { float *ln1_w, *ln1_b; void* qkv_w; float* qkv_b; void* so_w; float* so_b; float *ln2_w, *ln2_b;
                  void* cq_w; float* cq_b; void* co_w; float* co_b; float *ln3_w, *ln3_b; void* fc1_w; float* fc1_b;
                  void* fc2_w; float* fc2_b;
                  int qkv_q = 0, so_q = 0, cq_q = 0, co_q = 0, fc1_q = 0, fc2_q = 0; };
    void *conv1_w_, *conv2_w_, *ckv_w_, *tok_emb_;
    int tok_q_ = 0;
    int64_t res_weights_ = 0, res_bytes_ = 0;
    int res_type_ = -1;
    void plan_residency(const GgmlFile& f);
    float *conv1_b_, *conv2_b_, *enc_pos_, *lnp_w_, *lnp_b_, *ckv_b_, *dec_pos_, *lnf_w_, *lnf_b_;
    std::vector<EncL> enc_;
    std::vector<DecL> dec_;
    struct TRef { void* p; int64_t n; int dt; int q = 0; int64_t K = 0; };
    std::map<int, TRef> tref_;
    std::map<std::pair<int, int>, hipGraphExec_t> enc_graphs_;
    std::set<std::pair<int, int>> enc_seen_;

    float *hann_ = nullptr, *sinv_ = nullptr, *cosv_ = nullptr, *filt_ = nullptr;
    int* grp_ = nullptr;

    char* aarena_ = nullptr;
    int64_t abytes_ = 0;
    int *win_utt_ = nullptr, *win_seek_ = nullptr;
    void* mel_in_ = nullptr;
    void* y1p_ = nullptr;
    float* x_ = nullptr;
    void *xn_ = nullptr, *qkv_ = nullptr, *ao_ = nullptr, *ff_ = nullptr, *enc_out_ = nullptr;
    void* ckv_ = nullptr;
    uint32_t* suppress_ = nullptr;
    uint32_t* suppress_lang_ = nullptr;
    bool suppress_lang_ready_ = false;
    double* scratch_ = nullptr;
    float* zero_ = nullptr;
    std::vector<DecGroup> groups_;

    std::vector<uint32_t> host_suppress_;
    uint32_t suppress_flags_ = ~0u;
    std::vector<int> suppress_extra_;
    std::vector<int> ts_init_;
    DecodeRequest beam_rq_;
    int beam_B_ = 0;
    int beam_side_ = 0;
    void* kvtmp_ = nullptr;
    std::vector<int> beam_host_;
    std::vector<int> beam_tok_;
    std::vector<char> beam_rd_;
    void read_cands(int B, BeamCands* out);

    float* upcm_ = nullptr;
    int64_t upcm_cap_ = 0;
    float* umel_ = nullptr;
    int64_t umel_cap_ = 0;
    char* uinfo_ = nullptr;
    int uinfo_cap_ = 0;
    MelUtts mu_{};
    unsigned* umax_ = nullptr;
    std::vector<int> un_;
    std::vector<int64_t> uhost_;
    std::vector<char> mel_img_;
    std::vector<int> whost_;
    std::vector<int> kvrow_host_;
    int enc_E_ = 0;
// ... 13 lines not shown
```

spittle_amd/csrc/k_dec.hip:

```cpp
#include "common.h"
#include "ggml_qpack.h"
#include "kernels.h"

#include <stdio.h>
#include <stdlib.h>

#include <algorithm>
#include <type_traits>

#ifndef SPT_STAMP
#define SPT_STAMP 0
#endif

namespace spt {

#if SPT_STAMP
__device__ unsigned long long* g_xattn_stamp;
void set_xattn_stamp(void* p) { HIP_CHECK(hipMemcpyToSymbol(HIP_SYMBOL(g_xattn_stamp), &p, sizeof(p))); }
#define XA_STAMP(i)                                                                          \
    do {                                                                                     \
        if (g_xattn_stamp && threadIdx.x == 0)                                               \
            g_xattn_stamp[3 * blockIdx.x + (i)] = __builtin_amdgcn_s_memrealtime();          \
    } while (0)
#else
#define XA_STAMP(i) do {} while (0)
#endif

namespace {

template <typename T, bool QE = false>
__global__ void embed_kernel(const int* __restrict__ tok, int Tq, int d, const T* __restrict__ emb, int emb_q,
                             const float* __restrict__ pos, const DecState* __restrict__ ds, float* __restrict__ x) {
    const int r = blockIdx.x, t = r % Tq;
    const int p = ds->pos0 + t;
    const int tk = tok[r];
    const float* pp = pos + (size_t)p * d;
    for (int i = threadIdx.x; i < d; i += blockDim.x) x[(size_t)r * d + i] = emb_row_read<T, QE>(emb, emb_q, d, tk, i) + pp[i];
}

}
}

#include "dec_gemv.h"
#include "dec_attn.h"

namespace spt {
namespace {

template <typename T, int NQ, int NIX = 0>
__global__ __launch_bounds__(64 * AW) void self_attn_kernel(const T* __restrict__ q, int q_ld,
                                                            const T* __restrict__ kv, int B, int H, int ctx, int Tq,
                                                            const DecState* __restrict__ ds, T* __restrict__ out) {
    __shared__ float s_m[AW][NQ], s_l[AW][NQ];
    __shared__ float s_o[AW][NQ][64];
    const int bh = blockIdx.x, b = bh / H, h = bh - b * H;
    const int tid = threadIdx.x, lane = tid & 63, wid = tid >> 6, g = lane & 7;
    AttnWave<T, NQ, NIX> aw;
    aw.init(kv + (((size_t)0 * B + b) * H + h) * (size_t)ctx * 64 + 8 * g,
            kv + (((size_t)1 * B + b) * H + h) * (size_t)ctx * 64 + 8 * g, ctx, lane);
    aw.load_blk(aw.kc_[0], aw.vc_[0], wid);
    const int pos0 = ds->pos0;
    const int n_keys = pos0 + Tq;
    aw.n_keys = n_keys;
    float qv[NQ][8];
    int lim[NQ];
#pragma unroll
    for (int t = 0; t < NQ; ++t) {
        const int tt = t < Tq ? t : Tq - 1;
        const T* qr = q + (size_t)(b * Tq + tt) * q_ld + h * 64 + 8 * g;
#pragma unroll
        for (int e = 0; e < 8; ++e) qv[t][e] = to_f<T>(qr[e]) * kLog2Scale;
        lim[t] = pos0 + tt + 1;
    }
    aw.template run_pre<(448 / AttnWave<T, NQ, NIX>::KB + 1 + AW - 1) / AW>(wid, cdiv(n_keys, AttnWave<T, NQ, NIX>::KB), qv, lim, Tq);
    aw.to_lds(s_m, s_l, s_o, wid, lane);
    __syncthreads();
    if (tid < 64 * Tq) {
        const int t = tid >> 6, e = tid & 63;
        float M, L, O;
        attn_merge<NQ>(s_m, s_l, s_o, t, e, M, L, O);
        out[(size_t)(b * Tq + t) * (H * 64) + h * 64 + e] = from_f<T>(O / L);
    }
}

template <typename T, int NQ, bool SPLIT, int NW = AW, int NIX = 0, int PF = 2>
__global__ __launch_bounds__(64 * NW) void cross_attn_kernel(const T* __restrict__ q, const T* __restrict__ kv,
                                                             int B_layout, int H, int T_enc, int Tq,
                                                             T* __restrict__ out, float* __restrict__ part,
                                                             const int* __restrict__ kvrow, int share) {
    typedef AttnWave<T, NQ, NIX, NW, PF> W;
    XA_STAMP(0);
    __shared__ float s_m[NW][NQ], s_l[NW][NQ];
    __shared__ float s_o[NW][NQ][64];
    const int bh = blockIdx.x, j = bh / H, h = bh - j * H;
    const int tid = threadIdx.x, lane = tid & 63, wid = tid >> 6, g = lane & 7;
    const int nq_all = share * Tq;
    const int c0 = SPLIT ? 0 : (int)blockIdx.y * NQ;
    const int nq = min(NQ, nq_all - c0);
    const int kb = kvrow ? kvrow[j * share] : j;
    W aw;
    const size_t kvo = ((size_t)kb * H + h) * 4096 + 8 * g;
    aw.init(kv + kvo, kv + kvo + 2048, T_enc, lane, (int64_t)B_layout * H * 4096);
    const size_t qrow0 = (size_t)j * nq_all + c0;
    float qv[NQ][8];
    int lim[NQ];
#pragma unroll
    for (int t = 0; t < NQ; ++t) {
        const int tt = t < nq ? t : nq - 1;
        const T* qr = q + (qrow0 + tt) * (H * 64) + h * 64 + 8 * g;
#pragma unroll
        for (int e = 0; e < 8; ++e) qv[t][e] = to_f<T>(qr[e]) * kLog2Scale;
        lim[t] = T_enc;
    }
    const int nblk_all = cdiv(T_enc, W::KB);
    const int S = SPLIT ? (int)gridDim.y : 1, sp = SPLIT ? (int)blockIdx.y : 0;
    const int per = cdiv(nblk_all, S), blk0 = sp * per, nblk = min(nblk_all, blk0 + per);
    aw.template run<(1500 / W::KB + 1 + NW - 1) / NW>(blk0 + wid, nblk, qv, lim, nq);
    if (wid == 0) XA_STAMP(1);
    aw.to_lds(s_m, s_l, s_o, wid, lane);
    __syncthreads();
    XA_STAMP(2);
    for (int i = tid; i < 64 * nq; i += 64 * NW) {
        const int t = i >> 6, e = i & 63;
        float M, L, O;
        attn_merge<NQ, NW>(s_m, s_l, s_o, t, e, M, L, O);
        if constexpr (SPLIT) {
            float* pp = part + (((qrow0 + t) * H + h) * S + sp) * 66;
            pp[e] = O;
            if (e == 0) {
                pp[64] = M;
                pp[65] = L;
            }
        } else {
            out[(qrow0 + t) * (H * 64) + h * 64 + e] = from_f<T>(O / L);
        }
    }
}

template <typename T, int TOUCH, bool QW = false, int PF = 3>
__global__ __launch_bounds__(640) void xq_fused_kernel(GemvArgs a, XqFuseArgs x) {
    const int n_prod = a.N / 16;
    const unsigned tag =
        (__hip_atomic_load(&x.ds->epoch, __ATOMIC_RELAXED, __HIP_MEMORY_SCOPE_WORKGROUP) + 1u) * 64u + (unsigned)x.layer;
    if ((int)blockIdx.x < n_prod) {
        gemv_body<T, GV_BIAS, LN_SRC(0), 1, 10, 1, 1, true, true, QW>(a, x.gran, tag);
        return;
    }
    typedef AttnWave<T, 1, 0, AW, PF> W;
    constexpr int MAXB = (1500 / W::KB + 1 + AW - 1) / AW;
    extern __shared__ __attribute__((aligned(16))) char smem[];
    float (*s_o)[1][64] = (float (*)[1][64])smem;
    float (*s_m)[1] = (float (*)[1])(smem + AW * 256);
    float (*s_l)[1] = (float (*)[1])(smem + AW * 256 + AW * 4);
    unsigned short* s_q = (unsigned short*)(smem + AW * 256 + AW * 8);
    int* s_ok = (int*)(smem + AW * 256 + AW * 8 + 128);
    const int cb = (int)blockIdx.x - n_prod, j = cb / x.H, h = cb - j * x.H;
    const int tid = threadIdx.x, lane = tid & 63, wid = tid >> 6, g = lane & 7;
    if (wid > AW) return;
    const int nblk = cdiv(x.T_enc, W::KB);
    W aw;
    unsigned touch[TOUCH > 0 ? TOUCH : 1] = {};
    if (wid < AW) {
        const size_t kvo = ((size_t)j * x.H + h) * 4096 + 8 * g;
        aw.init((const T*)x.kv + kvo, (const T*)x.kv + kvo + 2048, x.T_enc, lane, (int64_t)x.B_layout * x.H * 4096);
        aw.template ring_fill<MAXB>(wid, nblk);
        if constexpr (TOUCH > 0) {
            const T* base = (const T*)x.kv + ((size_t)j * x.H + h) * 4096 + (lane < 32 ? 0 : 2048);
#pragma unroll
            for (int t = 0; t < TOUCH; ++t) {
                const int key = min((wid + (PF - 1 + t) * AW) * W::KB + (lane & 31), x.T_enc - 1);
                touch[t] = *(const unsigned*)(base + (uint32_t)((key >> 5) * aw.bstride + (key & 31) * 64));
            }
        }
    } else {
        unsigned long long* gp = x.gran + ((size_t)j * x.H + h) * 64 + lane;
        bool ok = false;
        if (__hip_atomic_load(x.err, __ATOMIC_RELAXED, __HIP_MEMORY_SCOPE_AGENT) == 0u) {
            const long long t0 = wall_clock64();
            for (;;) {
                const unsigned long long v = __hip_atomic_load(gp, __ATOMIC_RELAXED, __HIP_MEMORY_SCOPE_AGENT);
                if (__all((unsigned)(v >> 32) == tag)) {
                    s_q[lane] = (unsigned short)v;
                    ok = true;
                    break;
                }
                if (wall_clock64() - t0 > kXqTimeoutTicks) break;
                __builtin_amdgcn_s_sleep(2);
            }
        }
        if (lane == 0) {
            *s_ok = ok ? 1 : 0;
            if (!ok) __hip_atomic_store(x.err, 1u, __ATOMIC_RELAXED, __HIP_MEMORY_SCOPE_AGENT);
        }
    }
    __syncthreads();
    if (wid >= AW || !*s_ok) return;
    float qv[1][8];
    int lim[1] = {x.T_enc};
#pragma unroll
    for (int e = 0; e < 8; ++e) {
        T qt;
        __builtin_memcpy(&qt, &s_q[8 * g + e], 2);
        qv[0][e] = to_f<T>(qt) * kLog2Scale;
    }
    aw.template ring_run<MAXB>(wid, nblk, qv, lim, 1);
    aw.to_lds(s_m, s_l, s_o, wid, lane);
    __syncthreads();
    if (tid < 64) {
        float M, L, O;
        attn_merge<1, AW>(s_m, s_l, s_o, 0, tid, M, L, O);
        ((T*)x.out)[((size_t)j * x.H + h) * 64 + tid] = from_f<T>(O / L);
    }
    if constexpr (TOUCH > 0) {
        unsigned u = 0;
#pragma unroll
        for (int t = 0; t < TOUCH; ++t) u ^= touch[t];
        if (x.layer < 0 && u == 0x9e3779b9u) __hip_atomic_store(x.err, 2u, __ATOMIC_RELAXED, __HIP_MEMORY_SCOPE_AGENT);
    }
}

template <typename T, int NQ, int NIX = 0, int PF = 2>
__global__ __launch_bounds__(64) void cross_attn_vw_kernel(const T* __restrict__ q, const T* __restrict__ kv,
                                                           int B_layout, int H, int T_enc, int Tq,
                                                           float* __restrict__ part, const int* __restrict__ kvrow,
                                                           int share) {
    typedef AttnWave<T, NQ, NIX, AW, PF> W;
    __shared__ float s_m[1][NQ], s_l[1][NQ];
    __shared__ float s_o[1][NQ][64];
    const int bh = blockIdx.x, j = bh / H, h = bh - j * H;
    const int vw = blockIdx.y;
    const int lane = threadIdx.x, g = lane & 7;
    const int nq_all = share * Tq;
    const int c0 = (int)blockIdx.z * NQ;
    const int nq = min(NQ, nq_all - c0);
    const int kb = kvrow ? kvrow[j * share] : j;
    W aw;
    const size_t kvo = ((size_t)kb * H + h) * 4096 + 8 * g;
    aw.init(kv + kvo, kv + kvo + 2048, T_enc, lane, (int64_t)B_layout * H * 4096);
    const size_t qrow0 = (size_t)j * nq_all + c0;
    float qv[NQ][8];
    int lim[NQ];
#pragma unroll
    for (int t = 0; t < NQ; ++t) {
        const int tt = t < nq ? t : nq - 1;
        const T* qr = q + (qrow0 + tt) * (H * 64) + h * 64 + 8 * g;
#pragma unroll
        for (int e = 0; e < 8; ++e) qv[t][e] = to_f<T>(qr[e]) * kLog2Scale;
        lim[t] = T_enc;
    }
    aw.template run<(1500 / W::KB + 1 + AW - 1) / AW>(vw, cdiv(T_enc, W::KB), qv, lim, nq);
    aw.to_lds(s_m, s_l, s_o, 0, lane);
    __syncthreads();
    for (int i = lane; i < 64 * nq; i += 64) {
        const int t = i >> 6, e = i & 63;
        float* pp = part + (((qrow0 + t) * H + h) * AW + vw) * 66;
        pp[e] = s_o[0][t][e];
        if (e == 0) {
            pp[64] = s_m[0][t];
            pp[65] = s_l[0][t];
        }
    }
}

template <typename T>
__global__ __launch_bounds__(64) void attn_part_merge_kernel(const float* __restrict__ part, int H, T* __restrict__ out) {
#pragma clang fp contract(off)
    const int rh = blockIdx.x, e = threadIdx.x;
    const float* pp = part + (size_t)rh * AW * 66;
    float mw[AW], lw[AW], ow[AW];
#pragma unroll
    for (int w = 0; w < AW; ++w) {
        mw[w] = pp[w * 66 + 64];
        lw[w] = pp[w * 66 + 65];
        ow[w] = pp[w * 66 + e];
    }
    float M = -INFINITY;
#pragma unroll
    for (int w = 0; w < AW; ++w) M = fmaxf(M, mw[w]);
    float L = 0.f, O = 0.f;
#pragma unroll
    for (int w = 0; w < AW; ++w) {
        if (mw[w] == -INFINITY) continue;
        const float f = exp2f(mw[w] - M);
        L = __builtin_fmaf(lw[w], f, L);
        O = __builtin_fmaf(ow[w], f, O);
    }
    out[(size_t)rh * 64 + e] = from_f<T>(O / L);
}

constexpr int FIN_T = 1024;
template <typename T, bool QE = false>
__global__ __launch_bounds__(FIN_T) void finalize_kernel(FinalizeArgs a) {
    __shared__ TopP s_top[FIN_T / 64];
    __shared__ int s_tok;
    const int b = blockIdx.x, tid = threadIdx.x;
    const int step = a.ds->step, pos0 = a.ds->pos0;
    const unsigned epoch = a.ds->epoch;
    TopP t{-INFINITY, 0x7fffffff, -INFINITY, 0};
    const TopP* p = (const TopP*)a.part + (size_t)b * a.n_tiles;
    for (int i = tid; i < a.n_tiles; i += FIN_T) t = top_merge(t, p[i]);
#pragma unroll
    for (int o = 32; o > 0; o >>= 1) t = top_merge(t, top_shfl(t, o));
    if ((tid & 63) == 0) s_top[tid >> 6] = t;
    __syncthreads();
    if (tid == 0) {
        for (int w = 1; w < FIN_T / 64; ++w) t = top_merge(t, s_top[w]);
        if (t.i1 < 0 || t.i1 >= a.n_vocab) {
            t.i1 = -2;
            t.v1 = t.v2 = __builtin_nanf("");
        }
        int nxt = a.eot;
        if (step < a.out_cap) {
            const int oi = b * a.out_cap + step;
            if (a.done[b]) {
                a.out_tok[oi] = -1;
                a.out_top1[oi] = -INFINITY;
                a.out_top2[oi] = -INFINITY;
            } else {
                a.out_tok[oi] = t.i1;
                a.out_top1[oi] = t.v1;
                a.out_top2[oi] = t.v2;
                nxt = t.i1;
                if (a.forced && step < a.forced_len) nxt = a.forced[b * a.forced_len + step];
                if (!a.ignore_eot && t.i1 == a.eot) a.done[b] = 1;
                if (nxt < 0 || nxt >= a.n_vocab) nxt = a.eot;
            }
        }
        a.next_tok[b] = nxt;
        s_tok = nxt;
    }
    __syncthreads();
    const int tok = s_tok;
    const int pn = min(pos0 + a.Tq, a.ctx - 1);
    const float* pp = a.pos + (size_t)pn * a.d;
    for (int i = tid; i < a.d; i += FIN_T)
        a.x[(size_t)b * a.d + i] = emb_row_read<T, QE>(a.emb, a.emb_q, a.d, tok, i) + pp[i];
    if (tid == 0) {
        const unsigned prev = __hip_atomic_fetch_add(a.arrive, 1u, __ATOMIC_RELAXED, __HIP_MEMORY_SCOPE_AGENT);
        if (prev == (unsigned)gridDim.x - 1) {
            a.ds->pos0 = pos0 + a.Tq;
            a.ds->step = step + 1;
            a.ds->epoch = epoch + 1u;
            __hip_atomic_store(a.arrive, 0u, __ATOMIC_RELAXED, __HIP_MEMORY_SCOPE_AGENT);
        }
    }
}

__global__ void advance_kernel(DecState* ds, int n) {
    ds->pos0 += n;
    ds->epoch += 1u;
}

__global__ void reset_kernel(DecState* ds, unsigned* arrive) {
    ds->pos0 = 0;
    ds->step = 0;
    *arrive = 0u;
}

}

void gemv_prepare(int dtype) {
    if (dtype == DT_BF16) gemv_attr_modes<bf16>();
    else if (dtype == DT_F16) gemv_attr_modes<f16>();
    else gemv_attr_modes<float>();
}

int gemv_max_image_rows(int dtype, int K) {
    const int esz = dtype_size(dtype);
    int r = 64;
    while (r > 1 && gv_img_bytes(r, K, esz) > GV_LDS_BYTES) --r;
    return r;
}

void gemv(int dtype, int mode, int asrc, const GemvArgs& a_in, hipStream_t st) {
    if (a_in.R > 64 || a_in.R <= 0) throw std::runtime_error("gemv: rows must be in 1..64");
    const int ks = dtype_size(dtype) == 2 ? 128 : 64;
    if (a_in.K % ks) throw std::runtime_error("gemv: K alignment");
    GemvArgs a = a_in;
    a.ksplit = std::max(1, a.ksplit);
    if (a.ksplit > 1 && mode != GV_PARTIAL) throw std::runtime_error("gemv: K split needs partial outputs");
    if (a.ksplit > a.K / ks) throw std::runtime_error("gemv: K split exceeds the super-steps");
    const int esz = dtype_size(dtype);
    if (asrc != A_DIRECT && gv_img_bytes(a.R, a.K, esz) > GV_LDS_BYTES)
        throw std::runtime_error("gemv: A image exceeds the LDS budget");
    if (asrc == A_LN && (a.K > 1536 || !a.ln_w || !a.ln_b))
        throw std::runtime_error("gemv: LayerNorm prologue needs K <= 1536 and LN parameters");
    if (asrc == A_LN && (a.n_pend < 0 || a.n_pend > 4 || a.n_pend == 3))
        throw std::runtime_error("gemv: pending slab count must be 0, 1, 2 or 4");
    if (a.p_resid && mode != GV_PARTIAL) throw std::runtime_error("gemv: residual rows into slab 0 need partial outputs");
    if (asrc == A_LN)
        for (int p = 0; p < 4; ++p)
            if (!a.pend[p]) throw std::runtime_error("gemv: LayerNorm prologue needs 4 pending slabs (zero slab if none)");
    if (asrc == A_ATTN && (!a.apart || a.a_splits < 2 || (a.a_splits > 4 && a.a_splits != 8) || a.a_heads * 64 != a.K))
        throw std::runtime_error("gemv: attention-merge prologue needs 2..4 or 8 chunks over all heads");
    const int code = asrc == A_LN ? LN_SRC(a.n_pend) : asrc == A_ATTN ? ATTN_SRC(a.a_splits) : asrc;
    if (a.wq) {
        QPackGeom qg;
        if (esz != 2 || !qpack_geom(a.wq, &qg)) throw std::runtime_error("gemv: no resident layout for this weight type / dtype");
        gemv_q(dtype, mode, code, a, st);
        return;
    }
#define SPT_GV(M, S)                                                      \
    if (mode == M && code == S) {                                         \
        if (dtype == DT_BF16) gemv_launch<bf16, M, S>(a, st);             \
        else if (dtype == DT_F16) gemv_launch<f16, M, S>(a, st);          \
        else gemv_launch<float, M, S>(a, st);                             \
        return;                                                           \
    }
    SPT_GV_PAIRS(SPT_GV)
#undef SPT_GV
    throw std::runtime_error("gemv: unsupported mode / A source");
}

void dec_embed(int dtype, const int* tok, int R, int Tq, int d, const void* tok_emb, int tok_q, const float* pos_emb,
               const DecState* ds, float* x, hipStream_t st) {
    if (tok_q) {
        if (dtype == DT_BF16)
            hipLaunchKernelGGL((embed_kernel<bf16, true>), dim3(R), dim3(256), 0, st, tok, Tq, d, (const bf16*)tok_emb, tok_q, pos_emb, ds, x);
        else if (dtype == DT_F16)
            hipLaunchKernelGGL((embed_kernel<f16, true>), dim3(R), dim3(256), 0, st, tok, Tq, d, (const f16*)tok_emb, tok_q, pos_emb, ds, x);
        else throw std::runtime_error("dec_embed: a packed embedding needs a bf16 or f16 engine");
        return;
    }
    if (dtype == DT_BF16)
        hipLaunchKernelGGL(embed_kernel<bf16>, dim3(R), dim3(256), 0, st, tok, Tq, d, (const bf16*)tok_emb, 0, pos_emb, ds, x);
    else if (dtype == DT_F16)
        hipLaunchKernelGGL(embed_kernel<f16>, dim3(R), dim3(256), 0, st, tok, Tq, d, (const f16*)tok_emb, 0, pos_emb, ds, x);
    else
        hipLaunchKernelGGL(embed_kernel<float>, dim3(R), dim3(256), 0, st, tok, Tq, d, (const float*)tok_emb, 0, pos_emb, ds, x);
}

void dec_self_attn(int dtype, const void* q, const void* cache, int B, int H, int ctx, int Tq, const DecState* ds,
                   void* out, hipStream_t st) {
    if (Tq < 1 || Tq > 4) throw std::runtime_error("dec_self_attn: 1..4 queries per sequence");
    const dim3 grid(B * H), blk(64 * AW);
#define SPT_SA(T, NQ) \
    hipLaunchKernelGGL((self_attn_kernel<T, NQ>), grid, blk, 0, st, (const T*)q, H * 64, (const T*)cache, B, H, ctx, Tq, ds, (T*)out)
    if (dtype == DT_BF16) {
        if (Tq == 1) SPT_SA(bf16, 1); else SPT_SA(bf16, 4);
    } else if (dtype == DT_F16) {
        if (Tq == 1) SPT_SA(f16, 1); else SPT_SA(f16, 4);
    } else {
        if (Tq == 1) SPT_SA(float, 1); else SPT_SA(float, 4);
    }
#undef SPT_SA
    SPT_LAUNCH_CHECK();
}

static int xattn_pf() {
    static const int pf = getenv("SPT_XATTN_PF") ? std::max(2, std::min(4, atoi(getenv("SPT_XATTN_PF")))) : 2;
    return pf;
}

void dec_cross_attn(int dtype, const void* q, const void* kv, int B, int B_layout, int H, int T_enc, int Tq, void* out,
                    hipStream_t st, int splits, float* part, const int* kvrow, int share) {
    if (Tq < 1 || Tq > 4) throw std::runtime_error("dec_cross_attn: 1..4 queries per sequence");
    if (splits < 1 || splits > 4 || (splits > 1 && !part)) throw std::runtime_error("dec_cross_attn: 1..4 key chunks");
    if (share < 1 || share > 8 || B % share) throw std::runtime_error("dec_cross_attn: rows per window 1..8, dividing B");
    if (share > 1 && !kvrow) throw std::runtime_error("dec_cross_attn: shared windows need the window map");
    if ((int64_t)cdiv(T_enc, 32) * B_layout * H * 4096 >= (int64_t)INT32_MAX)
        throw std::runtime_error("dec_cross_attn: a layer's cross K/V exceeds 2^31 elements");
    const int nq = share * Tq;
    const int NQ = nq == 1 ? 1 : Tq > 1 ? 4 : (dtype_size(dtype) == 2 ? 5 : 4);
    if (splits > 1 && nq > NQ) throw std::runtime_error("dec_cross_attn: key chunks need one query chunk per window");
    const dim3 grid((B / share) * H, splits > 1 ? splits : cdiv(nq, NQ)), blk(64 * AW);
#define SPT_XA(T, NQ_, SP, NI, ...)                                                                             \
    hipLaunchKernelGGL((cross_attn_kernel<T, NQ_, SP, AW, NI __VA_ARGS__>), grid, blk, 0, st, (const T*)q,        \
                       (const T*)kv, B_layout, H, T_enc, Tq, (T*)out, part, kvrow, share)
#define SPT_XA_T(T)                                                                       \
    if (NQ == 1) {                                                                        \
        if (splits > 1) SPT_XA(T, 1, true, 0);                                            \
        else if (xattn_pf() == 4) SPT_XA(T, 1, false, 0, , 4);                            \
        else if (xattn_pf() == 3) SPT_XA(T, 1, false, 0, , 3);                            \
        else SPT_XA(T, 1, false, 0);                                                      \
    }                                                                                     \
    else if (NQ == 4 && Tq > 1) { if (splits > 1) SPT_XA(T, 4, true, 0); else SPT_XA(T, 4, false, 0); } \
    else if (NQ == 4) { if (splits > 1) SPT_XA(T, 4, true, 4); else SPT_XA(T, 4, false, 4); } \
    else { if (splits > 1) SPT_XA(T, 5, true, 4); else SPT_XA(T, 5, false, 4); }
    if (dtype == DT_BF16) { SPT_XA_T(bf16); }
    else if (dtype == DT_F16) { SPT_XA_T(f16); }
    else { SPT_XA_T(float); }
#undef SPT_XA_T
#undef SPT_XA
    SPT_LAUNCH_CHECK();
}

void dec_cross_attn_vw(int dtype, const void* q, const void* kv, int B, int B_layout, int H, int T_enc, int Tq,
                       float* part, hipStream_t st, const int* kvrow, int share, bool per_query) {
    if (Tq < 1 || Tq > 4) throw std::runtime_error("dec_cross_attn_vw: 1..4 queries per sequence");
    if (share < 1 || share > 8 || B % share) throw std::runtime_error("dec_cross_attn_vw: rows per window 1..8, dividing B");
    if (share > 1 && !kvrow) throw std::runtime_error("dec_cross_attn_vw: shared windows need the window map");
    if ((int64_t)cdiv(T_enc, 32) * B_layout * H * 4096 >= (int64_t)INT32_MAX)
        throw std::runtime_error("dec_cross_attn_vw: a layer's cross K/V exceeds 2^31 elements");
    if (!part) throw std::runtime_error("dec_cross_attn_vw: needs the partials buffer");
    const int nq = share * Tq;
    const int NQ = (nq == 1 || (per_query && Tq == 1)) ? 1 : Tq > 1 ? 4 : (dtype_size(dtype) == 2 ? 5 : 4);
    const dim3 grid((B / share) * H, AW, cdiv(nq, NQ)), blk(64);
#define SPT_XV(T, NQ_, NI, PF)                                                                               \
    hipLaunchKernelGGL((cross_attn_vw_kernel<T, NQ_, NI, PF>), grid, blk, 0, st, (const T*)q, (const T*)kv,      \
                       B_layout, H, T_enc, Tq, part, kvrow, share)
#define SPT_XV_PF(T, NQ_, NI)                                    \
    if (xattn_pf() == 4) SPT_XV(T, NQ_, NI, 4);                  \
    else if (xattn_pf() == 3) SPT_XV(T, NQ_, NI, 3);             \
    else SPT_XV(T, NQ_, NI, 2);
#define SPT_XV_T(T)                                         \
    if (NQ == 1) { SPT_XV_PF(T, 1, 0) }                     \
    else if (NQ == 4 && Tq > 1) SPT_XV(T, 4, 0, 2);         \
    else if (NQ == 4) SPT_XV(T, 4, 4, 2);                   \
    else { SPT_XV_PF(T, 5, 4) }
    if (dtype == DT_BF16) { SPT_XV_T(bf16); }
    else if (dtype == DT_F16) { SPT_XV_T(f16); }
    else { SPT_XV_T(float); }
#undef SPT_XV_T
#undef SPT_XV_PF
#undef SPT_XV
    SPT_LAUNCH_CHECK();
}

bool dec_xq_fused_ok(int dtype, int B, int d, int H, int T_enc, int n_cu) {
    static const bool exact_ln = !getenv("GV_EXACT_LN") || atoi(getenv("GV_EXACT_LN")) != 0;
    return exact_ln && dtype_size(dtype) == 2 && d == 10 * GV<bf16>::KS && H * 64 == d && B >= 1 && B <= 16 &&
           T_enc >= 256 && cdiv(T_enc, 32) <= 48 && d / 16 + B * H <= n_cu;
}

void dec_xq_fused(int dtype, const GemvArgs& cq, const XqFuseArgs& x, int B, hipStream_t st) {
    if (dtype_size(dtype) != 2 || cq.R != B || B < 1 || B > 16 || cq.N != x.H * 64 || cq.K != 10 * GV<bf16>::KS ||
        cq.N % 16 || cq.n_pend != 0 || !cq.ln_w || !cq.ln_b || !cq.C || x.T_enc < 256 || cdiv(x.T_enc, 32) > 48 ||
        x.layer < 0 || x.layer >= 64 || !x.kv || !x.out || !x.gran || !x.ds || !x.err)
        throw std::runtime_error("dec_xq_fused: not the fused launch's shape");
    for (int p = 0; p < 4; ++p)
        if (!cq.pend[p]) throw std::runtime_error("dec_xq_fused: LayerNorm prologue needs 4 pending slabs (zero slab if none)");
    if ((int64_t)cdiv(x.T_enc, 32) * x.B_layout * x.H * 4096 >= (int64_t)INT32_MAX)
        throw std::runtime_error("dec_xq_fused: a layer's cross K/V exceeds 2^31 elements");
    GemvArgs a = cq;
    a.ksplit = 1;
    const int lds = std::max(4096, gv_img_bytes(a.R, a.K, 2) + 10 * 64 * (int)sizeof(f32x4));
    const dim3 grid(a.N / 16 + B * x.H), blk(640);
    static const bool touch = !getenv("SPT_XQ_TOUCH") || atoi(getenv("SPT_XQ_TOUCH")) != 0;
    QPackGeom qg;
    if (a.wq && !qpack_geom(a.wq, &qg)) throw std::runtime_error("dec_xq_fused: no resident layout for this weight type");
#define SPT_XQ(T, TOUCH) \
    do { \
        if (a.wq) hipLaunchKernelGGL((xq_fused_kernel<T, TOUCH, true>), grid, blk, lds, st, a, x); \
        else hipLaunchKernelGGL((xq_fused_kernel<T, TOUCH>), grid, blk, lds, st, a, x); \
    } while (0)
    if (dtype == DT_BF16) {
        if (touch) SPT_XQ(bf16, 2);
        else SPT_XQ(bf16, 0);
    } else {
        if (touch) SPT_XQ(f16, 2);
        else SPT_XQ(f16, 0);
    }
#undef SPT_XQ
    SPT_LAUNCH_CHECK();
}

void dec_attn_part_merge(int dtype, const float* part, int R, int H, void* out, hipStream_t st) {
    if (R < 1 || H < 1 || !part || !out) throw std::runtime_error("dec_attn_part_merge: empty or missing buffers");
    if (dtype == DT_BF16) hipLaunchKernelGGL(attn_part_merge_kernel<bf16>, dim3(R * H), dim3(64), 0, st, part, H, (bf16*)out);
    else if (dtype == DT_F16) hipLaunchKernelGGL(attn_part_merge_kernel<f16>, dim3(R * H), dim3(64), 0, st, part, H, (f16*)out);
    else hipLaunchKernelGGL(attn_part_merge_kernel<float>, dim3(R * H), dim3(64), 0, st, part, H, (float*)out);
    SPT_LAUNCH_CHECK();
}

void dec_finalize(int dtype, const FinalizeArgs& a, int B, hipStream_t st) {
    if (a.emb_q) {
        if (dtype == DT_BF16) hipLaunchKernelGGL((finalize_kernel<bf16, true>), dim3(B), dim3(FIN_T), 0, st, a);
        else if (dtype == DT_F16) hipLaunchKernelGGL((finalize_kernel<f16, true>), dim3(B), dim3(FIN_T), 0, st, a);
        else throw std::runtime_error("dec_finalize: a packed embedding needs a bf16 or f16 engine");
        return;
    }
    if (dtype == DT_BF16) hipLaunchKernelGGL(finalize_kernel<bf16>, dim3(B), dim3(FIN_T), 0, st, a);
    else if (dtype == DT_F16) hipLaunchKernelGGL(finalize_kernel<f16>, dim3(B), dim3(FIN_T), 0, st, a);
    else hipLaunchKernelGGL(finalize_kernel<float>, dim3(B), dim3(FIN_T), 0, st, a);
}

void dec_advance(DecState* ds, int n, hipStream_t st) {
    hipLaunchKernelGGL(advance_kernel, dim3(1), dim3(1), 0, st, ds, n);
}

void dec_reset(DecState* ds, unsigned* arrive, hipStream_t st) {
    hipLaunchKernelGGL(reset_kernel, dim3(1), dim3(1), 0, st, ds, arrive);
}

}
```

spittle_amd/csrc/kernels.h:

```cpp
#pragma once
#include <hip/hip_runtime.h>
#include <stdint.h>

#include <string>

namespace spt {

enum { DT_F32 = 0, DT_BF16 = 1, DT_F16 = 2, DT_I8 = 3 };
inline int dtype_size(int dtype) { return dtype == DT_F32 ? 4 : 2; }

__host__ __device__ inline int64_t kv_layer_elems(int B, int H, int T) { return (int64_t)((T + 31) / 32) * B * H * 4096; }
__host__ __device__ inline int64_t kv_offset(int l, int kvi, int b, int h, int t, int e, int B, int H, int T) {
    return (int64_t)l * kv_layer_elems(B, H, T) + (((int64_t)(t >> 5) * B + b) * H + h) * 4096 + kvi * 2048 +
           (t & 31) * 64 + e;
}

enum { EPI_BIAS = 0, EPI_BIAS_GELU = 1, EPI_BIAS_GELU_POS = 2, EPI_BIAS_RESID = 3, EPI_KVSPLIT = 4,
       EPI_BIAS_SWISH = 5, EPI_BIAS_RELU = 6, EPI_BIAS_F32 = 7, EPI_PARTIAL = 8 };

struct GemmArgs {
    const void* A; int lda; int64_t sA;
    const void* W; int ldw;
    int M, N, K;
    const float* bias;
    void* C; int ldc; int64_t sC;
    const float* pos;
    int kv_B, kv_T, kv_H;
    float alpha = 1.0f;
    int ksplit = 1; int64_t c_split = 0;
    int nmajor = 0;
    int groups = 1;
};
void gemm_nt(int dtype, int epi, const GemmArgs& g, int batch, hipStream_t st);
void gemm_prepare();
void gemm_nt_variant(int dtype, int epi, const GemmArgs& g, int batch, int variant, hipStream_t st);

enum { WK_MAT = 0, WK_BIAS = 1, WK_LNW = 2, WK_LNB = 3, WK_TOK = 4, WK_DPOS = 5 };
void gen_weights(int store_dtype, void* dst, int64_t n, uint64_t seed, uint32_t tid, int kind,
                 int scale_exp, hipStream_t st);
void gen_conv_weights(int store_dtype, void* dst, int N, int C, int Cp, uint64_t seed, uint32_t tid,
                      int scale_exp, hipStream_t st);
void fill_f32(float* dst, int64_t n, float v, hipStream_t st);
void ggml_dequant(int type, const void* src, int64_t n, int out_dtype, void* dst, hipStream_t st);
void cache_flush(const void* p, int64_t bytes, unsigned* sink, hipStream_t st);
void set_xattn_stamp(void* p);
void dec_cross_attn_ni8(const void* q, const void* kv, int B, int B_layout, int H, int T_enc, void* out, int blocked,
                        hipStream_t st);
void stream_read(const void* p, int64_t bytes, unsigned* sink, int grid, int tpb, hipStream_t st);
void tensor_checksum(int dtype, const void* src, int64_t n, double* out2_dev, hipStream_t st);
void tensor_checksum_q(int dtype, int qtype, const void* packed, int64_t n, int64_t K, double* out2_dev, hipStream_t st);

struct MelTables {
    const float* hann;
    const float* sinv;
    const float* cosv;
    const float* filt;
    const int* grp;
};
constexpr int MEL_ROWS = 3002;
struct MelUtts {
    const int64_t* pcm_off;
    const int64_t* row_off;
    const int* n;
};
int mel_rows(int n);
void mel_frames(const float* pcm, MelUtts u, int U, int max_rows, int n_mels, MelTables t, float* mel_raw,
                unsigned* mel_max, hipStream_t st);
void mel_norm(int dtype, const float* mel_raw, const unsigned* mel_max, MelUtts u, const int* win_utt,
              const int* win_seek, int E, int n_mels, int Cp, void* mel_in, float* dbg, hipStream_t st);

void layernorm(int dtype, const float* x, int M, int d, const float* w, const float* b, void* y,
               hipStream_t st);
void layernorm_pend(int dtype, float* x, int M, int d, const float* slab, int ks, int64_t slab_stride,
                    const float* pbias, float alpha, const float* w, const float* b, void* y, bool write_x,
                    hipStream_t st);
void layernorm_pend2(int dtype2, const float* x, int M, int d, const float* slab, int ks, int64_t slab_stride,
                     const float* pbias, float alpha, const float* w, const float* b, float* y, const float* w2,
                     const float* b2, void* y2, hipStream_t st);
void to_f32(int dtype, const void* src, float* dst, int64_t n, hipStream_t st);

void enc_attention(int dtype, const void* qkv, int B, int T, int H, void* out, hipStream_t st);

struct DecState {
    int pos0;
    int step;
    unsigned epoch;
};

enum { GV_BIAS = 0, GV_BIAS_GELU = 1, GV_PARTIAL = 2, GV_QKV_CACHE = 3, GV_LOGITS = 4, GV_BIAS_RESID = 5 };
enum { A_DIRECT = 0, A_LN = 1, A_ATTN = 2 };
struct GemvArgs {
    const void* A; int lda; int a_row0;
    const float* ln_w; const float* ln_b;
    const float* pend[4]; int n_pend;
    float* x_out;
    const float* apart; int a_splits, a_heads;
    int R;
    int wq;
    const void* W; int N, K;
    const float* bias;
    void* C; int ldc;
    int ksplit; int64_t c_split;
    const float* p_resid;
    void* cache; int cache_B, cache_H, cache_ctx, Tq;
    const DecState* st;
    const uint32_t* suppress; int blank0, blank1;
    void* part; int n_tiles;
    unsigned long long* stamp;
};
constexpr int kMaxPend = 4;
void gemv(int dtype, int mode, int asrc, const GemvArgs& a, hipStream_t st);
void gemv_prepare(int dtype);
void gemv_q(int dtype, int mode, int code, const GemvArgs& a, hipStream_t st);
void gemv_q_prepare(int dtype);
int gemv_max_image_rows(int dtype, int K);

void dec_embed(int dtype, const int* tok, int R, int Tq, int d, const void* tok_emb, int tok_q,
               const float* pos_emb, const DecState* ds, float* x, hipStream_t st);
void dec_self_attn(int dtype, const void* q, const void* cache, int B, int H, int ctx, int Tq,
                   const DecState* ds, void* out, hipStream_t st);
void dec_cross_attn(int dtype, const void* q, const void* kv, int B, int B_layout, int H, int T_enc, int Tq,
                    void* out, hipStream_t st, int splits = 1, float* part = nullptr, const int* kvrow = nullptr,
                    int share = 1);
void dec_cross_attn_vw(int dtype, const void* q, const void* kv, int B, int B_layout, int H, int T_enc, int Tq,
                       float* part, hipStream_t st, const int* kvrow = nullptr, int share = 1, bool per_query = false);
struct XqFuseArgs {
    const void* kv; int B_layout, H, T_enc;
    void* out;
    unsigned long long* gran;
    const DecState* ds;
    unsigned* err;
    int layer;
};
constexpr long long kXqTimeoutTicks = 2000000;
bool dec_xq_fused_ok(int dtype, int B, int d, int H, int T_enc, int n_cu);
void dec_xq_fused(int dtype, const GemvArgs& cq, const XqFuseArgs& x, int B, hipStream_t st);

void dec_attn_part_merge(int dtype, const float* part, int R, int H, void* out, hipStream_t st);

struct FinalizeArgs {
    const void* part; int n_tiles;
    int eot; int ignore_eot; int n_vocab;
    const int* forced; int forced_len;
    int* next_tok;
    int* out_tok; float* out_top1; float* out_top2; int out_cap;
    int* done;
    const void* emb; const float* pos; int d, ctx, Tq;
    float* x;
    DecState* ds; unsigned* arrive;
    int emb_q;
};
void dec_finalize(int dtype, const FinalizeArgs& a, int B, hipStream_t st);
void dec_reset(DecState* ds, unsigned* arrive, hipStream_t st);



struct TsParams {
    float temperature;
    int suppress_blank;
    int no_ts;
    int max_initial;
    int n_max;
    int max_tokens;
    unsigned long long seed;
};
struct TsArgs {
    const float* logits; int ldl;
    int n_vocab, eot, beg, blank;
    const uint32_t* suppress;
    const TsParams* prm;
    const int* seek; const int* seek_end;
    int* state;
    const int* forced; int forced_len;
    int* next_tok;
    int* out_tok; float* out_plog; float* out_tid; int out_cap;
    int* done;
    const void* emb; const float* pos; int d, ctx, Tq;
    float* x;
    DecState* ds; unsigned* arrive;
    float* stat;
    int emb_q;
};
constexpr int TS_CHUNKS = 16;
void dec_ts_stats(const TsArgs& a, int B, hipStream_t st);
void dec_finalize_ts(int dtype, const TsArgs& a, int B, hipStream_t st);
struct BeamArgs {
    const float* logits; int ldl;
    int n_vocab, eot, beg, blank;
    const uint32_t* suppress;
    const TsParams* prm;
    const int* row;
    const int* step;
    int k;
    int* cand_id; float* cand_lp;
    int* tid;
    float* stat;
};
constexpr int BEAM_STAT = 6 + 4 * 8;
void dec_beam_topk(const BeamArgs& a, int B, hipStream_t st);
void dec_kv_gather(int dtype, const void* src, void* dst, const int* rows, int L, int B, int H, int ctx,
                   const DecState* ds, hipStream_t st);
void dec_advance(DecState* ds, int n, hipStream_t st);

}
```

spittle_amd/csrc/ubench.cpp:

```cpp
#include <hip/hip_runtime.h>
#include <stdio.h>
#include <stdlib.h>
#include <string.h>

#include <algorithm>
#include <functional>
#include <string>
#include <vector>

#include "common.h"
#include "kernels.h"

using namespace spt;

static void* dalloc(size_t bytes) {
    void* p;
    HIP_CHECK(hipMalloc(&p, bytes));
    HIP_CHECK(hipMemset(p, 0, bytes));
    return p;
}
static void* drand(size_t n, int dt, uint32_t tid, int e) {
    void* p = dalloc(n * (dtype_size(dt)));
    gen_weights(dt, p, (int64_t)n, 7, tid, WK_MAT, e, 0);
    return p;
// ... 199 lines not shown
        const int esz = dtype_size(dt);
        void* W = drand((size_t)N * K, dt, 1, -5);
        float* bias = frand(N, 2, -5);
        float* lnw = frand(K, 3, -3);
        float* lnb = frand(K, 4, -4);
        void* A = ln ? (void*)frand((size_t)R * K, 5, 0) : drand((size_t)R * K, dt, 5, 0);
        float* zero = (float*)dalloc((size_t)4 * R * K * 4);
        void* C = dalloc((size_t)4 * R * N * 4 + 64);
        void* cache = dalloc((size_t)2 * R * 20 * 448 * 64 * esz);
        uint32_t* sup = (uint32_t*)dalloc(N / 8 + 64);
        void* part = dalloc((size_t)R * ((N + 15) / 16) * 16 + 64);
        GemvArgs a{};
        a.A = A; a.lda = K; a.R = R; a.W = W; a.N = N; a.K = K; a.bias = bias; a.C = C; a.ldc = N;
        if (ln) { a.ln_w = lnw; a.ln_b = lnb; }
        for (int p = 0; p < kMaxPend; ++p) a.pend[p] = zero + (size_t)p * R * K;
        a.n_pend = npend;
        a.cache = cache; a.cache_B = R; a.cache_H = N / 3 / 64; a.cache_ctx = 448; a.Tq = 1; a.st = ds;
        a.suppress = sup; a.blank0 = a.blank1 = -1; a.part = part; a.n_tiles = (N + 15) / 16;
        a.ksplit = ksplit; a.c_split = (int64_t)R * N;
        if (mode == GV_QKV_CACHE) a.ldc = N / 3;
        const double us = time_us(st, iters, [&] { gemv(dt, mode, ln ? A_LN : A_DIRECT, a, st); });
        const double bytes = (double)N * K * esz;
        printf("gemv N=%d K=%d R=%d mode=%d ln=%d dt=%d ksplit=%d npend=%d : %.2f us  %.0f GB/s\n", N, K, R, mode, ln, dt,
               ksplit, npend, us, bytes / us / 1e3);
        return 0;
    }
    if (what == "attn") {
        const int B = ai(2, 8), H = ai(3, 20), ctx = ai(4, 448), nk = ai(5, 132), Tq = ai(6, 1), dt = ai(7, DT_BF16);
        const int esz = dtype_size(dt);
        void* q = drand((size_t)B * Tq * H * 64, dt, 1, 0);
        void* kv = drand((size_t)2 * B * H * ctx * 64, dt, 2, 0);
        void* out = dalloc((size_t)B * Tq * H * 64 * esz);
        DecState h{nk - Tq, 0};
        HIP_CHECK(hipMemcpy(ds, &h, sizeof(h), hipMemcpyHostToDevice));
        const double us = time_us(st, iters, [&] { dec_self_attn(dt, q, kv, B, H, ctx, Tq, ds, out, st); });
        printf("self-attn B=%d H=%d nk=%d Tq=%d dt=%d : %.2f us  %.0f GB/s\n", B, H, nk, Tq, dt, us,
               2.0 * B * H * nk * 64 * esz / us / 1e3);
        return 0;
    }
    if (what == "xattn") {
        const int B = ai(2, 8), T = ai(3, 1500), S = ai(4, 1), dt = ai(5, DT_BF16), NL = 8, d = 1280, H = 20;
        const int esz = dtype_size(dt);
        void* q = drand((size_t)B * d, dt, 1, 0);
        const size_t layer = (size_t)2 * B * H * ((T + 31) / 32 * 32) * 64;
        void* kv = drand(layer * NL, dt, 2, 0);
        void* out = dalloc((size_t)B * d * esz);
        float* part = (float*)dalloc((size_t)B * H * 32 * 66 * 4);
        HIP_CHECK(hipDeviceSynchronize());
        const double us = time_us(st, 10, [&] {
            for (int l = 0; l < NL; ++l) dec_cross_attn(dt, q, (const char*)kv + layer * l * esz, B, B, H, T, 1, out, st, S, part);
        }) / NL;
#if SPT_STAMP
        {
            unsigned long long* sp = (unsigned long long*)dalloc((size_t)B * H * 3 * 8);
            void* flush = dalloc((size_t)512 << 20);
            unsigned* sink = (unsigned*)dalloc(64);
            cache_flush(flush, (int64_t)512 << 20, sink, st);
            set_xattn_stamp(sp);
            dec_cross_attn(dt, q, kv, B, B, H, T, 1, out, st, S, part);
            HIP_CHECK(hipStreamSynchronize(st));
            set_xattn_stamp(nullptr);
            std::vector<unsigned long long> h((size_t)B * H * 3);
            HIP_CHECK(hipMemcpy(h.data(), sp, h.size() * 8, hipMemcpyDeviceToHost));
            unsigned long long t0 = ~0ull;
            for (int i = 0; i < B * H; ++i) t0 = std::min(t0, h[3 * i]);
            std::vector<double> st_, str_, end_;
            for (int i = 0; i < B * H; ++i) {
                st_.push_back((h[3 * i] - t0) * 0.01);
                str_.push_back((h[3 * i + 1] - t0) * 0.01);
                end_.push_back((h[3 * i + 2] - t0) * 0.01);
            }
            auto q5 = [](std::vector<double> v) {
                std::sort(v.begin(), v.end());
                char b[128];
                snprintf(b, sizeof b, "min %.2f med %.2f max %.2f", v.front(), v[v.size() / 2], v.back());
                return std::string(b);
            };
            printf("  timeline us from first start: start %s | wave0 streamed %s | merged %s\n", q5(st_).c_str(),
                   q5(str_).c_str(), q5(end_).c_str());
        }
#endif
        printf("cross-attn B=%d T=%d splits=%d dt=%d (8 layers back to back) : %.2f us  %.0f GB/s\n", B, T, S, dt, us,
               2.0 * B * H * T * 64 * esz / us / 1e3);
        return 0;
    }
    if (what == "gemm") {
        const int M = ai(2, 12000), N = ai(3, 5120), K = ai(4, 1280), epi = ai(5, 0), dt = ai(6, DT_BF16), ks = ai(7, 1);
        void* A = drand((size_t)M * K, dt, 1, -2);
        void* W = drand((size_t)N * K, dt, 2, -5);
        float* bias = frand(N, 3, -5);
        const size_t cbytes = (size_t)ks * M * N * 4;
        void* C = dalloc(cbytes);
        float* C0 = frand(cbytes / 4, 5, 0);
        GemmArgs g{};
        g.alpha = 1.0f;
        g.A = A; g.lda = K; g.W = W; g.ldw = K; g.M = M; g.N = N; g.K = K; g.bias = bias; g.C = C; g.ldc = N;
        g.kv_B = M / 1500; g.kv_T = 1500; g.kv_H = 20; g.ksplit = ks; g.c_split = (int64_t)M * N;
        if (epi == EPI_BIAS_GELU_POS) g.pos = frand((size_t)M * N, 4, 0);
        HIP_CHECK(hipDeviceSynchronize());
        std::vector<char> ref(cbytes), out(cbytes);
        double us[7] = {0, 0, 0, 0, 0, 0, 0};
        std::vector<char> out64(cbytes), out6464(cbytes), outring(cbytes);
        const bool ring = dt != DT_F32 && N % 64 == 0;
        for (int v : {1, 2, 4, 5, 6}) {
            if (v == 6 && !ring) continue;
            HIP_CHECK(hipMemcpyAsync(C, C0, cbytes, hipMemcpyDeviceToDevice, st));
            gemm_nt_variant(dt, epi, g, 1, v, st);
            HIP_CHECK(hipStreamSynchronize(st));
            HIP_CHECK(hipMemcpy(v == 1 ? ref.data() : v == 2 ? out.data() : v == 4 ? out64.data() : v == 5 ? out6464.data() : outring.data(),
                                C, cbytes, hipMemcpyDeviceToHost));
            us[v] = time_us(st, 20, [&] { gemm_nt_variant(dt, epi, g, 1, v, st); });
        }
        size_t diff64 = 0, diff6464 = 0, diffring = 0;
        for (size_t i = 0; i < cbytes; ++i) {
            diff64 += ref[i] != out64[i];
            diff6464 += ref[i] != out6464[i];
            diffring += ring && ref[i] != outring[i];
        }
        if (ring) printf("ring 208x64: %.2f us %.1f TF/s, bytes differing from 128-tile %zu\n", us[6], 2.0 * M * N * K / us[6] / 1e6, diffring);
        size_t diff = 0, shown = 0;
        for (size_t i = 0; i < cbytes; ++i) {
            if (ref[i] == out[i]) continue;
            ++diff;
            if (shown < 6 && epi == EPI_KVSPLIT && (i & 1) == 0) {
                const size_t e = i / 2, el = e % 64, t = e / 64 % 1500, h = e / 64 / 1500 % 20, bb = e / 64 / 1500 / 20 % g.kv_B,
                             lk = e / 64 / 1500 / 20 / g.kv_B;
                const size_t row = bb * 1500 + t, col = (lk / 2) * 2560 + (lk % 2) * 1280 + h * 64 + el;
                printf("  diff at row %zu col %zu: 128=%04x 256=%04x\n", row, col, ((uint16_t*)ref.data())[e], ((uint16_t*)out.data())[e]);
                ++shown;
            }
        }
        const double fl = 2.0 * M * N * K;
        printf("gemm M=%d N=%d K=%d ks=%d epi=%d dt=%d : 128-tile %.2f us %.1f TF/s | 256-tile %.2f us %.1f TF/s | bytes differing %zu"
               " | 64x128 %.2f us %.1f TF/s, bytes differing from 128-tile %zu | 64x64 %.2f us, differing %zu\n",
               M, N, K, ks, epi, dt, us[1], fl / us[1] / 1e6, us[2], fl / us[2] / 1e6, diff, us[4], fl / us[4] / 1e6, diff64,
               us[5], diff6464);
        return 0;
    }
    if (what == "layer" || what == "layer2") {
        const int B = ai(2, 8), dt = ai(3, DT_BF16), xs = ai(4, 1), d = 1280, H = 20, ctx = 448, T = 1500;
        gemv_prepare(dt);
        const int esz = dtype_size(dt);
        void* wqkv = drand((size_t)3 * d * d, dt, 1, -4);
        void* wo = drand((size_t)d * d, dt, 2, -4);
        void* wq = drand((size_t)d * d, dt, 3, -4);
        void* wco = drand((size_t)d * d, dt, 4, -4);
        void* w1 = drand((size_t)4 * d * d, dt, 5, -4);
        void* w2 = drand((size_t)4 * d * d, dt, 6, -5);
        float* b4 = frand(4 * d, 7, -5);
        float* lnw = frand(d, 8, -3);
        float* lnb = frand(d, 9, -4);
        float* zero = (float*)dalloc((size_t)B * d * 4);
        struct Chain { float *x, *x2, *pend, *xpart; void *q, *ao, *ff, *skv, *ckv; DecState* ds; };
        auto mk = [&](uint32_t s) {
            Chain c;
            c.x = frand((size_t)B * d, 10 + s, 0);
            c.x2 = (float*)dalloc((size_t)B * d * 4);
            c.pend = (float*)dalloc((size_t)kMaxPend * B * d * 4);
            c.xpart = (float*)dalloc((size_t)B * H * 4 * 66 * 4);
            c.q = dalloc((size_t)B * d * esz);
            c.ao = dalloc((size_t)B * d * esz);
            c.ff = dalloc((size_t)B * 4 * d * esz);
            c.skv = drand((size_t)2 * B * H * ctx * 64, dt, 11 + s, 0);
            c.ckv = drand((size_t)2 * B * H * T * 64, dt, 12 + s, 0);
            c.ds = (DecState*)dalloc(64);
            DecState h{128, 0};
// ... 112 lines not shown
```

Before: 985.1 audio-sec/wall-sec.

## Stage cross-attention KV blocks into LDS via spare wave while Q gemv runs

In the fused cross-Q/cross-attention kernel, the otherwise idle extra wave of each consumer workgroup now prefetches the first blocks of each attention wave's K/V into LDS using global_load_lds while consumers wait for the Q producers. The attention waves then consume the staged blocks before resuming their register-prefetch pipeline. The default also turns off the L2 'touch' prefetch and selects the kernel variant from a table keyed by these settings. This raises LDS use per workgroup and adds barriers, which could reduce residency or add sync cost in a persistent, spin-waiting launch.

```diff
diff --git a/include/spittle_hip.h b/include/spittle_hip.h
--- a/include/spittle_hip.h
+++ b/include/spittle_hip.h
@@ -207,6 +207,10 @@
                                 const float* v, float pad_value, int32_t B, int32_t B_layout, int32_t b0, int32_t H,
                                 int32_t T_enc, int32_t Tq, int32_t splits, const int32_t* kvrow, int32_t share,
                                 float* out, float* part, char* err, size_t errlen);
+spt_status spt_debug_xq_fused(int32_t device, int32_t dtype, const float* x, const float* ln_w, const float* ln_b,
+                              const float* wq, const float* bias, const float* k, const float* v, float pad_value,
+                              int32_t B, int32_t H, int32_t T_enc, int32_t lds, int32_t touch, float* q, float* out,
+                              char* err, size_t errlen);
 
 #define SPT_HAS_QUANT_RESIDENT 1
 spt_status spt_get_weight_residency(const spt_ctx* ctx, int64_t* resident_weights, int64_t* resident_bytes,
diff --git a/rust/spittle-hip-sys/src/lib.rs b/rust/spittle-hip-sys/src/lib.rs
--- a/rust/spittle-hip-sys/src/lib.rs
+++ b/rust/spittle-hip-sys/src/lib.rs
@@ -394,6 +394,27 @@
         err: *mut c_char,
         errlen: usize,
     ) -> spt_status;
+    pub fn spt_debug_xq_fused(
+        device: i32,
+        dtype: i32,
+        x: *const f32,
+        ln_w: *const f32,
+        ln_b: *const f32,
+        wq: *const f32,
+        bias: *const f32,
+        k: *const f32,
+        v: *const f32,
+        pad_value: f32,
+        b: i32,
+        h: i32,
+        t_enc: i32,
+        lds: i32,
+        touch: i32,
+        q: *mut f32,
+        out: *mut f32,
+        err: *mut c_char,
+        errlen: usize,
+    ) -> spt_status;
     pub fn spt_get_weight_residency(
         ctx: *const spt_ctx,
         resident_weights: *mut i64,
diff --git a/spittle_amd/_lib.py b/spittle_amd/_lib.py
--- a/spittle_amd/_lib.py
+++ b/spittle_amd/_lib.py
@@ -44,7 +44,7 @@
     "spt_sensevoice_transcribe_batch", "spt_sensevoice_result_free", "spt_sensevoice_get_timings",
     "spt_sensevoice_debug_features", "spt_sensevoice_debug_encode", "spt_sensevoice_debug_frames",
     "spt_debug_sample_tokens", "spt_debug_sample_beam", "spt_debug_sample_kv_gather",
-    "spt_debug_attn_enc", "spt_debug_attn_self", "spt_debug_attn_cross",
+    "spt_debug_attn_enc", "spt_debug_attn_self", "spt_debug_attn_cross", "spt_debug_xq_fused",
     "spt_debug_qgemv", "spt_get_weight_residency",
 ]
 SPT_MODEL_QUANT_RESIDENT = 2
@@ -404,7 +404,9 @@
     L.spt_debug_attn_self.argtypes = [i32, i32, fp, fp, i32, i32, i32, i32, i32, fp, C.c_char_p, C.c_size_t]
     L.spt_debug_attn_cross.argtypes = [i32, i32, i32, fp, fp, fp, C.c_float, i32, i32, i32, i32, i32, i32, i32, i32p,
                                        i32, fp, fp, C.c_char_p, C.c_size_t]
-    for fn in ("spt_debug_attn_enc", "spt_debug_attn_self", "spt_debug_attn_cross"):
+    L.spt_debug_xq_fused.argtypes = [i32, i32, fp, fp, fp, fp, fp, fp, fp, C.c_float, i32, i32, i32, i32, i32, fp, fp,
+                                     C.c_char_p, C.c_size_t]
+    for fn in ("spt_debug_attn_enc", "spt_debug_attn_self", "spt_debug_attn_cross", "spt_debug_xq_fused"):
         getattr(L, fn).restype = C.c_int
     L.spt_debug_qgemv.argtypes = [i32, i32, i32, C.c_void_p, C.c_size_t, i32, i32, fp, i32, fp, fp, fp, fp, i32, i32,
                                   i32, fp, fp, fp, fp, fp, C.c_char_p, C.c_size_t]
diff --git a/spittle_amd/attn_debug.py b/spittle_amd/attn_debug.py
--- a/spittle_amd/attn_debug.py
+++ b/spittle_amd/attn_debug.py
@@ -75,3 +75,23 @@
                                   b0, H, T_enc, Tq, splits, _ptr(km, C.c_int32), share, _ptr(out), _ptr(part), err, 512)
     _check(st, err)
     return part if want_part else out
+
+
+def xq_fused(x, ln_w, ln_b, wq, bias, k, v, *, lds=0, touch=2, pad_value=0.0, dtype="bf16", H=None, device: int = 0):
+    lib = L.load()
+    f = lambda a: None if a is None else np.ascontiguousarray(a, np.float32)
+    xx, kk, vv = f(x), f(k), f(v)
+    B = xx.shape[0] if xx is not None else kk.shape[0]
+    if H is None:
+        H = kk.shape[1]
+    T_enc = kk.shape[2]
+    if kk.shape != (B, H, T_enc, 64) or (vv is not None and vv.shape != kk.shape):
+        raise ValueError("xq_fused: k and v are [B][H][T_enc][64]")
+    q = np.zeros((max(B, 1), 1280), np.float32)
+    out = np.zeros((max(B, 1), 1280), np.float32)
+    err = C.create_string_buffer(512)
+    st = lib.spt_debug_xq_fused(device, DTYPES[dtype], _ptr(xx), _ptr(f(ln_w)), _ptr(f(ln_b)), _ptr(f(wq)), _ptr(f(bias)),
+                                _ptr(kk), _ptr(vv), float(pad_value), B, H, T_enc, int(lds), int(touch), _ptr(q), _ptr(out),
+                                err, 512)
+    _check(st, err)
+    return q, out
diff --git a/spittle_amd/csrc/capi_attn.cpp b/spittle_amd/csrc/capi_attn.cpp
--- a/spittle_amd/csrc/capi_attn.cpp
+++ b/spittle_amd/csrc/capi_attn.cpp
@@ -195,4 +195,83 @@
     }
 }
 
-}
+spt_status spt_debug_xq_fused(int32_t device, int32_t dtype, const float* x, const float* ln_w, const float* ln_b,
+                              const float* wq, const float* bias, const float* k, const float* v, float pad_value,
+                              int32_t B, int32_t H, int32_t T_enc, int32_t lds, int32_t touch, float* q, float* out,
+                              char* err, size_t errlen) {
+    if (!x || !ln_w || !ln_b || !wq || !bias || !k || !v || !q || !out) {
+        set_err(err, errlen, "null argument");
+        return SPT_ERR_INVALID_ARG;
+    }
+    const int d = 1280;
+    try {
+        if (dtype != spt::DT_BF16 && dtype != spt::DT_F16) throw std::runtime_error("debug_xq_fused: dtype is bf16 or f16");
+        if (H != d / 64) throw std::runtime_error("debug_xq_fused: the fused launch is d = 1280, H = 20");
+        if (B < 1 || B > 16) throw std::runtime_error("debug_xq_fused: 1..16 rows");
+        if (T_enc < 256 || T_enc > 1536) throw std::runtime_error("debug_xq_fused: T_enc in 256..1536");
+        if (lds < 0 || lds > 2) throw std::runtime_error("debug_xq_fused: 0..2 staged blocks per wave");
+        if (touch != 0 && touch != 2) throw std::runtime_error("debug_xq_fused: 0 or 2 touched blocks per wave");
+    } catch (const std::exception& e) {
+        set_err(err, errlen, e.what());
+        return SPT_ERR_INVALID_ARG;
+    }
+    if (spt_status s = device_ok(device, err, errlen)) return s;
+    try {
+        hipDeviceProp_t prop;
+        HIP_CHECK(hipGetDeviceProperties(&prop, device));
+        if (!spt::dec_xq_fused_ok(dtype, B, d, H, T_enc, prop.multiProcessorCount)) {
+            set_err(err, errlen, "debug_xq_fused: 80 + B * H workgroups are not all resident on this device");
+            return SPT_ERR_INVALID_ARG;
+        }
+        const size_t n_kv = (size_t)spt::kv_layer_elems(B, H, T_enc);
+        std::vector<float> lay(n_kv, pad_value);
+        const int T32 = (T_enc + 31) / 32 * 32;
+        for (int kvi = 0; kvi < 2; ++kvi) {
+            const float* src = kvi ? v : k;
+            for (int b = 0; b < B; ++b)
+                for (int h = 0; h < H; ++h)
+                    for (int t = 0; t < T32; ++t) {
+                        float* dst = lay.data() + spt::kv_offset(0, kvi, b, h, t, 0, B, H, T_enc);
+                        if (t < T_enc) memcpy(dst, src + (((size_t)b * H + h) * T_enc + t) * 64, 64 * sizeof(float));
+                    }
+        }
+        const size_t nq = (size_t)B * d, esz = (size_t)spt::dtype_size(dtype);
+        const spt::DecState ds0{0, 0, 0u};
+        std::vector<uint16_t> w16, kv16;
+        Scope sc(device);
+        spt::gemv_prepare(dtype);
+        float* zero = sc.alloc<float>(nq);
+        HIP_CHECK(hipMemsetAsync(zero, 0, nq * sizeof(float), sc.st));
+        unsigned long long* gran = sc.alloc<unsigned long long>(nq);
+        HIP_CHECK(hipMemsetAsync(gran, 0, nq * sizeof(unsigned long long), sc.st));
+        unsigned* werr = sc.alloc<unsigned>(1);
+        HIP_CHECK(hipMemsetAsync(werr, 0, sizeof(unsigned), sc.st));
+        spt::GemvArgs a{};
+        a.A = sc.up(x, nq); a.lda = d; a.R = B;
+        a.ln_w = sc.up(ln_w, (size_t)d); a.ln_b = sc.up(ln_b, (size_t)d);
+        for (int p = 0; p < spt::kMaxPend; ++p) a.pend[p] = zero;
+        a.W = up_as(sc, dtype, wq, (size_t)d * d, w16); a.N = d; a.K = d;
+        a.bias = sc.up(bias, (size_t)d);
+        a.C = sc.out<char>(nq * esz); a.ldc = d;
+        spt::XqFuseArgs xa{};
+        xa.kv = up_as(sc, dtype, lay.data(), n_kv, kv16); xa.B_layout = B; xa.H = H; xa.T_enc = T_enc;
+        xa.out = sc.out<char>(nq * esz); xa.gran = gran; xa.ds = sc.up(&ds0, 1); xa.err = werr; xa.layer = 0;
+        xa.lds = lds; xa.touch = touch;
+        spt::dec_xq_fused(dtype, a, xa, B, sc.st);
+        unsigned herr = 0;
+        sc.down(&herr, (const unsigned*)werr, 1);
+        down_f32(sc, dtype, a.C, q, nq);
+        down_f32(sc, dtype, xa.out, out, nq);
+        sc.sync();
+        if (herr) {
+            set_err(err, errlen, "debug_xq_fused: a consumer's wait for q ran out");
+            return SPT_ERR_DEVICE;
+        }
+        return SPT_OK;
+    } catch (const std::exception& e) {
+        set_err(err, errlen, e.what());
+        return spt_classify(e);
+    }
+}
+
+}
diff --git a/spittle_amd/csrc/dec_attn.h b/spittle_amd/csrc/dec_attn.h
--- a/spittle_amd/csrc/dec_attn.h
+++ b/spittle_amd/csrc/dec_attn.h
@@ -174,6 +174,41 @@
             process(kc_[i % PF], vc_[i % PF], (blk + i * NW) * KB, qv, lim, Tq);
         }
     }
+    template <int MAXB, int NS>
+    __device__ __forceinline__ void staged_head(int blk, int nblk, const float (&qv)[NQ][8], const int (&lim)[NQ], int Tq) {
+        static_assert(PF == 3 && NI == 4 && sizeof(T) == 2 && NS >= 1 && 2 + NS <= MAXB && MAXB <= 8,
+                      "AttnWave: the staged schedule is the fused launch's");
+        const int cnt = blk < nblk ? (nblk - 1 - blk) / NW + 1 : 0;
+        const int mine = blk + (max(cnt, 1) - 1) * NW;
+#pragma unroll
+        for (int p = 0; p < 2; ++p) {
+            if (p + 2 < MAXB - NS) load_blk(kc_[(p + 2) % PF], vc_[(p + 2) % PF], min(blk + (p + 2 + NS) * NW, mine));
+            if (p < cnt) process(kc_[p], vc_[p], (blk + p * NW) * KB, qv, lim, Tq);
+        }
+    }
+    template <int MAXB, int NS>
+    __device__ __forceinline__ void staged_tail(int blk, int nblk, const float (&qv)[NQ][8], const int (&lim)[NQ], int Tq,
+                                                const char* st) {
+        if (blk >= nblk) return;
+        const int cnt = (nblk - 1 - blk) / NW + 1;
+        const int mine = blk + (cnt - 1) * NW;
+#pragma unroll
+        for (int s = 0; s < NS; ++s) {
+            if (2 + s >= cnt) return;
+#pragma unroll
+            for (int i = 0; i < NI; ++i) {
+                kc_[1][i].load((const T*)(st + s * 8192 + i * 1024));
+                vc_[1][i].load((const T*)(st + s * 8192 + 4096 + i * 1024));
+            }
+            process(kc_[1], vc_[1], (blk + (2 + s) * NW) * KB, qv, lim, Tq);
+        }
+#pragma unroll
+        for (int p = 2; p < MAXB - NS; ++p) {
+            if (p + NS >= cnt) return;
+            if (p + 2 < MAXB - NS) load_blk(kc_[(p + 2) % PF], vc_[(p + 2) % PF], min(blk + (p + 2 + NS) * NW, mine));
+            process(kc_[p % PF], vc_[p % PF], (blk + (p + NS) * NW) * KB, qv, lim, Tq);
+        }
+    }
     __device__ __forceinline__ void to_lds(float (*s_m)[NQ], float (*s_l)[NQ], float (*s_o)[NQ][64], int wid,
                                            int lane) {
         const int g = lane & 7;
diff --git a/spittle_amd/csrc/engine.cpp b/spittle_amd/csrc/engine.cpp
--- a/spittle_amd/csrc/engine.cpp
+++ b/spittle_amd/csrc/engine.cpp
@@ -980,7 +980,7 @@
             if (np != 0) throw std::runtime_error("fused cross-Q launch: pending slabs before LN2");
             XqFuseArgs x{};
             x.kv = ckv_l; x.B_layout = E; x.H = H; x.T_enc = T; x.out = g.dao; x.gran = g.xq_gran; x.ds = g.ds;
-            x.err = xq_err_; x.layer = l;
+            x.err = xq_err_; x.layer = l; x.lds = xq_lds_; x.touch = xq_touch_;
             dec_xq_fused(dt_, a, x, B, st);
         } else {
             gemv(dt_, GV_BIAS, A_LN, a, st);
@@ -1295,7 +1295,7 @@
         for (DecGroup* g : act) {
             GraphKey key{g->B, E, g->b0, out_cap, rq.n_forced, rq.flags, rq.full};
             key.share = S;
-            key.fuse = xq_on_;
+            key.fuse = xq_on_ ? 1 + xq_lds_ + 4 * xq_touch_ : 0;
             auto it = g->graphs.find(key);
             if (it == g->graphs.end()) {
                 hipGraph_t graph;
@@ -1348,6 +1348,10 @@
     require_weights();
     const char* xq_env = getenv("SPT_XQ_FUSE");
     xq_on_ = rq.beam_k == 0 && !(xq_env && atoi(xq_env) == 0);
+    const char* lds_env = getenv("SPT_XQ_LDS");
+    xq_lds_ = lds_env ? std::min(2, std::max(0, atoi(lds_env))) : kXqLdsDefault;
+    const char* touch_env = getenv("SPT_XQ_TOUCH");
+    xq_touch_ = touch_env ? (atoi(touch_env) != 0 ? 2 : 0) : kXqTouchDefault;
     struct XqOff {
         bool& on;
         ~XqOff() { on = false; }
diff --git a/spittle_amd/csrc/engine.h b/spittle_amd/csrc/engine.h
--- a/spittle_amd/csrc/engine.h
+++ b/spittle_amd/csrc/engine.h
@@ -112,7 +112,7 @@
         uint32_t flags;
         bool full;
         int share = 0;
-        bool fuse = false;
+        int fuse = 0;
         bool operator<(const GraphKey& o) const {
             if (full != o.full) return full < o.full;
             if (fuse != o.fuse) return fuse < o.fuse;
@@ -192,6 +192,7 @@
     bool pend_fold_ = true;
     void ln_source(GemvArgs& a, float* xc, float* pend, int np, int64_t slab) const;
     bool xq_on_ = false;
+    int xq_lds_ = kXqLdsDefault, xq_touch_ = kXqTouchDefault;
     int xq_enq_ = 0;
     int n_cu_ = 0;
     unsigned* xq_err_ = nullptr;
diff --git a/spittle_amd/csrc/k_dec.hip b/spittle_amd/csrc/k_dec.hip
--- a/spittle_amd/csrc/k_dec.hip
+++ b/spittle_amd/csrc/k_dec.hip
@@ -22,8 +22,16 @@
         if (g_xattn_stamp && threadIdx.x == 0)                                               \
             g_xattn_stamp[3 * blockIdx.x + (i)] = __builtin_amdgcn_s_memrealtime();          \
     } while (0)
+__device__ unsigned long long* g_xq_stamp;
+void set_xq_stamp(void* p) { HIP_CHECK(hipMemcpyToSymbol(HIP_SYMBOL(g_xq_stamp), &p, sizeof(p))); }
+#define XQ_STAMP(i)                                                                          \
+    do {                                                                                     \
+        if (g_xq_stamp && threadIdx.x == 0)                                                  \
+            g_xq_stamp[5 * blockIdx.x + (i)] = __builtin_amdgcn_s_memrealtime();             \
+    } while (0)
 #else
 #define XA_STAMP(i) do {} while (0)
+#define XQ_STAMP(i) do {} while (0)
 #endif
 
 namespace {
@@ -137,13 +145,16 @@
     }
 }
 
-template <typename T, int TOUCH, bool QW = false, int PF = 3>
+constexpr int kXqStage = 4096;
+template <typename T, int TOUCH, bool QW = false, int LDSB = 0, int PF = 3>
 __global__ __launch_bounds__(640) void xq_fused_kernel(GemvArgs a, XqFuseArgs x) {
     const int n_prod = a.N / 16;
     const unsigned tag =
         (__hip_atomic_load(&x.ds->epoch, __ATOMIC_RELAXED, __HIP_MEMORY_SCOPE_WORKGROUP) + 1u) * 64u + (unsigned)x.layer;
+    XQ_STAMP(0);
     if ((int)blockIdx.x < n_prod) {
         gemv_body<T, GV_BIAS, LN_SRC(0), 1, 10, 1, 1, true, true, QW>(a, x.gran, tag);
+        XQ_STAMP(4);
         return;
     }
     typedef AttnWave<T, 1, 0, AW, PF> W;
@@ -156,8 +167,35 @@
     int* s_ok = (int*)(smem + AW * 256 + AW * 8 + 128);
     const int cb = (int)blockIdx.x - n_prod, j = cb / x.H, h = cb - j * x.H;
     const int tid = threadIdx.x, lane = tid & 63, wid = tid >> 6, g = lane & 7;
-    if (wid > AW) return;
     const int nblk = cdiv(x.T_enc, W::KB);
+    if (wid > AW) {
+        if constexpr (LDSB > 0) {
+            typedef const __attribute__((address_space(1))) void* GP;
+            typedef __attribute__((address_space(3))) void* LP;
+            const T* kb = (const T*)x.kv + ((size_t)j * x.H + h) * 4096 + 8 * g;
+            const int bstride = x.B_layout * x.H * 4096, slot = lane >> 3;
+#pragma unroll
+            for (int s = 0; s < LDSB; ++s) {
+#pragma unroll
+                for (int w = 0; w < AW; ++w) {
+                    const int mine = w + (nblk - 1 - w) / AW * AW;
+                    const int blk = min(w + (2 + s) * AW, mine);
+#pragma unroll
+                    for (int i = 0; i < W::NI; ++i) {
+                        const int key = min(blk * W::KB + 8 * i + slot, x.T_enc - 1);
+                        const uint32_t off = (uint32_t)((key >> 5) * bstride + (key & 31) * 64);
+                        char* dst = smem + kXqStage + ((w * LDSB + s) * 8 + i) * 1024;
+                        __builtin_amdgcn_global_load_lds((GP)(kb + off), (LP)dst, 16, 0, 0);
+                        __builtin_amdgcn_global_load_lds((GP)(kb + 2048 + off), (LP)(dst + 4096), 16, 0, 0);
+                    }
+                }
+            }
+            asm volatile("s_barrier" ::: "memory");
+            asm volatile("s_waitcnt vmcnt(0)" ::: "memory");
+            if (__builtin_amdgcn_readfirstlane(*s_ok)) asm volatile("s_barrier" ::: "memory");
+        }
+        return;
+    }
     W aw;
     unsigned touch[TOUCH > 0 ? TOUCH : 1] = {};
     if (wid < AW) {
@@ -195,6 +233,7 @@
     }
     __syncthreads();
     if (wid >= AW || !*s_ok) return;
+    XQ_STAMP(1);
     float qv[1][8];
     int lim[1] = {x.T_enc};
 #pragma unroll
@@ -203,7 +242,15 @@
         __builtin_memcpy(&qt, &s_q[8 * g + e], 2);
         qv[0][e] = to_f<T>(qt) * kLog2Scale;
     }
-    aw.template ring_run<MAXB>(wid, nblk, qv, lim, 1);
+    if constexpr (LDSB > 0) {
+        aw.template staged_head<MAXB, LDSB>(wid, nblk, qv, lim, 1);
+        asm volatile("s_barrier" ::: "memory");
+        XQ_STAMP(2);
+        aw.template staged_tail<MAXB, LDSB>(wid, nblk, qv, lim, 1, smem + kXqStage + wid * LDSB * 8192 + lane * 16);
+    } else {
+        aw.template ring_run<MAXB>(wid, nblk, qv, lim, 1);
+    }
+    XQ_STAMP(3);
     aw.to_lds(s_m, s_l, s_o, wid, lane);
     __syncthreads();
     if (tid < 64) {
@@ -211,6 +258,7 @@
         attn_merge<1, AW>(s_m, s_l, s_o, 0, tid, M, L, O);
         ((T*)x.out)[((size_t)j * x.H + h) * 64 + tid] = from_f<T>(O / L);
     }
+    XQ_STAMP(4);
     if constexpr (TOUCH > 0) {
         unsigned u = 0;
 #pragma unroll
@@ -360,6 +408,7 @@
 }
 
 void gemv_prepare(int dtype) {
+    dec_xq_fused_prepare(dtype);
     if (dtype == DT_BF16) gemv_attr_modes<bf16>();
     else if (dtype == DT_F16) gemv_attr_modes<f16>();
     else gemv_attr_modes<float>();
@@ -517,6 +566,30 @@
     SPT_LAUNCH_CHECK();
 }
 
+namespace {
+typedef void (*XqKernel)(GemvArgs, XqFuseArgs);
+template <typename T>
+XqKernel xq_kernel(int touch, bool qw, int ldsb) {
+#define SPT_XQ_L(TO, QW) {xq_fused_kernel<T, TO, QW, 0>, xq_fused_kernel<T, TO, QW, 1>, xq_fused_kernel<T, TO, QW, 2>}
+    static const XqKernel tab[2][2][3] = {{SPT_XQ_L(0, false), SPT_XQ_L(0, true)}, {SPT_XQ_L(2, false), SPT_XQ_L(2, true)}};
+#undef SPT_XQ_L
+    return tab[touch ? 1 : 0][qw ? 1 : 0][ldsb];
+}
+int xq_lds_bytes(int R, int K, int ldsb) {
+    const int prod = std::max(4096, gv_img_bytes(R, K, 2) + 10 * 64 * (int)sizeof(f32x4));
+    return std::max(prod, ldsb > 0 ? kXqStage + AW * ldsb * 8192 : 0);
+}
+}
+
+void dec_xq_fused_prepare(int dtype) {
+    if (dtype_size(dtype) != 2) return;
+    for (int touch = 0; touch <= 2; touch += 2)
+        for (int qw = 0; qw < 2; ++qw)
+            for (int l = 1; l <= 2; ++l)
+                ensure_lds_attr((const void*)(dtype == DT_BF16 ? xq_kernel<bf16>(touch, qw, l) : xq_kernel<f16>(touch, qw, l)),
+                                xq_lds_bytes(16, 1280, l));
+}
+
 bool dec_xq_fused_ok(int dtype, int B, int d, int H, int T_enc, int n_cu) {
     static const bool exact_ln = !getenv("GV_EXACT_LN") || atoi(getenv("GV_EXACT_LN")) != 0;
     return exact_ln && dtype_size(dtype) == 2 && d == 10 * GV<bf16>::KS && H * 64 == d && B >= 1 && B <= 16 &&
@@ -534,24 +607,13 @@
         throw std::runtime_error("dec_xq_fused: a layer's cross K/V exceeds 2^31 elements");
     GemvArgs a = cq;
     a.ksplit = 1;
-    const int lds = std::max(4096, gv_img_bytes(a.R, a.K, 2) + 10 * 64 * (int)sizeof(f32x4));
+    if (x.lds < 0 || x.lds > 2 || (x.touch != 0 && x.touch != 2))
+        throw std::runtime_error("dec_xq_fused: 0..2 staged blocks, 0 or 2 touched blocks");
     const dim3 grid(a.N / 16 + B * x.H), blk(640);
-    static const bool touch = !getenv("SPT_XQ_TOUCH") || atoi(getenv("SPT_XQ_TOUCH")) != 0;
     QPackGeom qg;
     if (a.wq && !qpack_geom(a.wq, &qg)) throw std::runtime_error("dec_xq_fused: no resident layout for this weight type");
-#define SPT_XQ(T, TOUCH) \
-    do { \
-        if (a.wq) hipLaunchKernelGGL((xq_fused_kernel<T, TOUCH, true>), grid, blk, lds, st, a, x); \
-        else hipLaunchKernelGGL((xq_fused_kernel<T, TOUCH>), grid, blk, lds, st, a, x); \
-    } while (0)
-    if (dtype == DT_BF16) {
-        if (touch) SPT_XQ(bf16, 2);
-        else SPT_XQ(bf16, 0);
-    } else {
-        if (touch) SPT_XQ(f16, 2);
-        else SPT_XQ(f16, 0);
-    }
-#undef SPT_XQ
+    const XqKernel k = dtype == DT_BF16 ? xq_kernel<bf16>(x.touch, a.wq != 0, x.lds) : xq_kernel<f16>(x.touch, a.wq != 0, x.lds);
+    hipLaunchKernelGGL(k, grid, blk, xq_lds_bytes(a.R, a.K, x.lds), st, a, x);
     SPT_LAUNCH_CHECK();
 }
 
diff --git a/spittle_amd/csrc/kernels.h b/spittle_amd/csrc/kernels.h
--- a/spittle_amd/csrc/kernels.h
+++ b/spittle_amd/csrc/kernels.h
@@ -44,6 +44,7 @@
 void ggml_dequant(int type, const void* src, int64_t n, int out_dtype, void* dst, hipStream_t st);
 void cache_flush(const void* p, int64_t bytes, unsigned* sink, hipStream_t st);
 void set_xattn_stamp(void* p);
+void set_xq_stamp(void* p);
 void dec_cross_attn_ni8(const void* q, const void* kv, int B, int B_layout, int H, int T_enc, void* out, int blocked,
                         hipStream_t st);
 void stream_read(const void* p, int64_t bytes, unsigned* sink, int grid, int tpb, hipStream_t st);
@@ -131,10 +132,14 @@
     const DecState* ds;
     unsigned* err;
     int layer;
-};
+    int lds = 0;
+    int touch = 2;
+};
+constexpr int kXqLdsDefault = 1, kXqTouchDefault = 0;
 constexpr long long kXqTimeoutTicks = 2000000;
 bool dec_xq_fused_ok(int dtype, int B, int d, int H, int T_enc, int n_cu);
 void dec_xq_fused(int dtype, const GemvArgs& cq, const XqFuseArgs& x, int B, hipStream_t st);
+void dec_xq_fused_prepare(int dtype);
 
 void dec_attn_part_merge(int dtype, const float* part, int R, int H, void* out, hipStream_t st);
 
diff --git a/spittle_amd/csrc/ubench.cpp b/spittle_amd/csrc/ubench.cpp
--- a/spittle_amd/csrc/ubench.cpp
+++ b/spittle_amd/csrc/ubench.cpp
@@ -305,6 +305,78 @@
 #endif
         printf("cross-attn B=%d T=%d splits=%d dt=%d (8 layers back to back) : %.2f us  %.0f GB/s\n", B, T, S, dt, us,
                2.0 * B * H * T * 64 * esz / us / 1e3);
+        return 0;
+    }
+    if (what == "xqfused") {
+        const int B = ai(2, 8), T = ai(3, 1500), lds = ai(4, 0), touch = ai(5, 2), dt = ai(6, DT_BF16), NL = 8, d = 1280, H = 20;
+        const int esz = dtype_size(dt);
+        gemv_prepare(dt);
+        const size_t layer = (size_t)2 * B * H * ((T + 31) / 32 * 32) * 64;
+        void* kv = drand(layer * NL, dt, 2, 0);
+        void* W = drand((size_t)d * d * NL, dt, 3, -5);
+        float* bias = frand(d, 4, -5);
+        float* lnw = frand(d, 5, -3);
+        float* lnb = frand(d, 6, -4);
+        float* x = frand((size_t)B * d, 7, 0);
+        float* zero = (float*)dalloc((size_t)B * d * 4);
+        void* q = dalloc((size_t)B * d * esz);
+        void* out = dalloc((size_t)B * d * esz);
+        unsigned long long* gran = (unsigned long long*)dalloc((size_t)B * d * 8);
+        unsigned* err = (unsigned*)dalloc(64);
+        auto launch = [&](int l) {
+            GemvArgs a{};
+            a.A = x; a.lda = d; a.R = B; a.ln_w = lnw; a.ln_b = lnb;
+            for (int p = 0; p < kMaxPend; ++p) a.pend[p] = zero;
+            a.W = (const char*)W + (size_t)d * d * l * esz; a.N = d; a.K = d; a.bias = bias; a.C = q; a.ldc = d;
+            XqFuseArgs xa{};
+            xa.kv = (const char*)kv + layer * l * esz; xa.B_layout = B; xa.H = H; xa.T_enc = T; xa.out = out; xa.gran = gran;
+            xa.ds = ds; xa.err = err; xa.layer = l; xa.lds = lds; xa.touch = touch;
+            dec_xq_fused(dt, a, xa, B, st);
+        };
+        HIP_CHECK(hipDeviceSynchronize());
+        const double us = time_us(st, 10, [&] {
+            for (int l = 0; l < NL; ++l) launch(l);
+            dec_advance(ds, 1, st);
+        }) / NL;
+#if SPT_STAMP
+        {
+            const int n_prod = d / 16, nwg = n_prod + B * H;
+            unsigned long long* sp = (unsigned long long*)dalloc((size_t)nwg * 5 * 8);
+            void* flush = dalloc((size_t)512 << 20);
+            unsigned* sink = (unsigned*)dalloc(64);
+            cache_flush(flush, (int64_t)512 << 20, sink, st);
+            HIP_CHECK(hipStreamSynchronize(st));
+            set_xq_stamp(sp);
+            launch(0);
+            HIP_CHECK(hipStreamSynchronize(st));
+            set_xq_stamp(nullptr);
+            std::vector<unsigned long long> h((size_t)nwg * 5);
+            HIP_CHECK(hipMemcpy(h.data(), sp, h.size() * 8, hipMemcpyDeviceToHost));
+            unsigned long long t0 = ~0ull;
+            for (int i = 0; i < nwg; ++i) t0 = std::min(t0, h[5 * i]);
+            auto q3 = [&](int w0, int w1, int k) {
+                std::vector<double> v;
+                for (int i = w0; i < w1; ++i)
+                    if (h[5 * i + k]) v.push_back((h[5 * i + k] - t0) * 0.01);
+                char b[128] = "-";
+                if (!v.empty()) {
+                    std::sort(v.begin(), v.end());
+                    snprintf(b, sizeof b, "%.2f / %.2f / %.2f", v.front(), v[v.size() / 2], v.back());
+                }
+                return std::string(b);
+            };
+            printf("  timeline, us from the first workgroup's entry (min / median / max over workgroups):\n");
+            printf("    producers (%d): entry %s | exit %s\n", n_prod, q3(0, n_prod, 0).c_str(), q3(0, n_prod, 4).c_str());
+            printf("    consumers (%d): entry %s | q seen %s | staged blocks ready %s | streamed %s | exit %s\n", B * H,
+                   q3(n_prod, nwg, 0).c_str(), q3(n_prod, nwg, 1).c_str(), q3(n_prod, nwg, 2).c_str(),
+                   q3(n_prod, nwg, 3).c_str(), q3(n_prod, nwg, 4).c_str());
+        }
+#endif
+        unsigned herr = 0;
+        HIP_CHECK(hipMemcpy(&herr, err, 4, hipMemcpyDeviceToHost));
+        printf("xq-fused B=%d T=%d lds=%d touch=%d dt=%d (8 layers back to back, one advance per 8) : %.2f us  %.0f GB/s%s\n",
+               B, T, lds, touch, dt, us, (2.0 * B * H * T * 64 + (double)d * d) * esz / us / 1e3,
+               herr ? "  [a consumer's wait ran out]" : "");
         return 0;
     }
     if (what == "gemm") {
```

After: 998.4 audio-sec/wall-sec, median of 6. 1.01x the previous value.
